# DIYer22/calibrating

Measured on AMD Instinct MI355X. Metric: stereo pairs/s at 1920x1080 numDisparities=128, higher is better.
Workload: dtype int16; 1 GPU; cv2.StereoSGBM-equivalent disparity of 1920x1080 rectified RGB pairs, numDisparities=128 blockSize=5 mode=MODE_SGBM(5 paths), median3 on, speckle off; batches_in_flight_per_gpu=2, parallelism=pairs sharded over 1 GPU(s), no data-path collective

## Files before the change

### calibrating_amd/csrc/common.hpp

```cpp
#pragma once

#include <hip/hip_runtime.h>

#include <cstdarg>
#include <cstdint>
#include <cstdio>

#include "../../include/calibrating_amd.h"
#include "../../include/calibrating_amd_experimental.h"

namespace camd {

void set_error(const char* fmt, ...);

#define CAMD_HIP(call)                                                                  \
    do {                                                                                \
        hipError_t e_ = (call);                                                         \
        if (e_ != hipSuccess) {                                                         \
            camd::set_error("%s failed: %s (%s:%d)", #call, hipGetErrorString(e_),      \
                            __FILE__, __LINE__);                                        \
            return CAMD_ERR_HIP;                                                        \
        }                                                                               \
    } while (0)

#define CAMD_LAUNCH_CHECK()                                                             \
    do {                                                                                \
        hipError_t e_ = hipGetLastError();                                              \
        if (e_ != hipSuccess) {                                                         \
            camd::set_error("kernel launch failed: %s (%s:%d)", hipGetErrorString(e_),  \
                            __FILE__, __LINE__);                                        \
            return CAMD_ERR_HIP;                                                        \
        }                                                                               \
    } while (0)

typedef unsigned short u16x2_t __attribute__((ext_vector_type(2)));
typedef short s16x2_t __attribute__((ext_vector_type(2)));

__device__ __forceinline__ uint32_t pk_min_u16(uint32_t a, uint32_t b)
{
    return __builtin_bit_cast(uint32_t, __builtin_elementwise_min(__builtin_bit_cast(u16x2_t, a),
                                                                  __builtin_bit_cast(u16x2_t, b)));
}
__device__ __forceinline__ uint32_t pk_max_u16(uint32_t a, uint32_t b)
{
    return __builtin_bit_cast(uint32_t, __builtin_elementwise_max(__builtin_bit_cast(u16x2_t, a),
                                                                  __builtin_bit_cast(u16x2_t, b)));
}
__device__ __forceinline__ uint32_t pk_add_u16(uint32_t a, uint32_t b)
{
    return __builtin_bit_cast(uint32_t, __builtin_bit_cast(u16x2_t, a) + __builtin_bit_cast(u16x2_t, b));
}
__device__ __forceinline__ uint32_t pk_sub_u16(uint32_t a, uint32_t b)
{
    return __builtin_bit_cast(uint32_t, __builtin_bit_cast(u16x2_t, a) - __builtin_bit_cast(u16x2_t, b));
}
__device__ __forceinline__ uint32_t pk_min_i16(uint32_t a, uint32_t b)
{
    return __builtin_bit_cast(uint32_t, __builtin_elementwise_min(__builtin_bit_cast(s16x2_t, a),
                                                                  __builtin_bit_cast(s16x2_t, b)));
}
__device__ __forceinline__ uint32_t pk_max_i16(uint32_t a, uint32_t b)
{
    return __builtin_bit_cast(uint32_t, __builtin_elementwise_max(__builtin_bit_cast(s16x2_t, a),
                                                                  __builtin_bit_cast(s16x2_t, b)));
}
__device__ __forceinline__ uint32_t pk_subsat_u16(uint32_t a, uint32_t b)
{
    return __builtin_bit_cast(uint32_t, __builtin_elementwise_sub_sat(__builtin_bit_cast(u16x2_t, a),
                                                                      __builtin_bit_cast(u16x2_t, b)));
}
__device__ __forceinline__ uint32_t pk_addsat_i16(uint32_t a, uint32_t b)
{
    return __builtin_bit_cast(uint32_t, __builtin_elementwise_add_sat(__builtin_bit_cast(s16x2_t, a),
                                                                      __builtin_bit_cast(s16x2_t, b)));
}
__device__ __forceinline__ uint32_t pk_subsat_i16(uint32_t a, uint32_t b)
{
    return __builtin_bit_cast(uint32_t, __builtin_elementwise_sub_sat(__builtin_bit_cast(s16x2_t, a),
                                                                      __builtin_bit_cast(s16x2_t, b)));
}
__device__ __forceinline__ uint32_t pk_mad_sat_u16(uint32_t a, uint32_t b, uint32_t c)
{
    uint32_t r;
    asm("v_pk_mad_u16 %0, %1, %2, %3 clamp" : "=v"(r) : "v"(a), "v"(b), "v"(c));
    return r;
}
__device__ __forceinline__ uint32_t pk_lshr_u16(uint32_t a, uint32_t sh_pk)
{
    return __builtin_bit_cast(uint32_t, __builtin_bit_cast(u16x2_t, a) >> __builtin_bit_cast(u16x2_t, sh_pk));
}
__device__ __forceinline__ uint32_t alignbit16(uint32_t hi, uint32_t lo)
{
    return __builtin_amdgcn_alignbit(hi, lo, 16);
}
__device__ __forceinline__ uint32_t dup16(uint32_t v) { return (v & 0xffffu) | (v << 16); }

enum : int {
    DPP_QUAD_XOR1 = 0xB1,
    DPP_QUAD_XOR2 = 0x4E,
    DPP_ROW_SHL1 = 0x101,
    DPP_ROW_SHR1 = 0x111,
    DPP_WAVE_SHL1 = 0x130,
    DPP_WAVE_SHR1 = 0x138,
    DPP_ROW_MIRROR = 0x140,
    DPP_ROW_HALF_MIRROR = 0x141
};

template <int CTRL>
__device__ __forceinline__ uint32_t dpp_mov(uint32_t old, uint32_t src)
{
    return (uint32_t)__builtin_amdgcn_update_dpp((int)old, (int)src, CTRL, 0xf, 0xf, false);
}

template <int LANES>
__device__ __forceinline__ uint32_t group_min_pk_u16(uint32_t v)
{
    if (LANES >= 2) v = pk_min_u16(v, dpp_mov<DPP_QUAD_XOR1>(v, v));
    if (LANES >= 4) v = pk_min_u16(v, dpp_mov<DPP_QUAD_XOR2>(v, v));
    if (LANES >= 8) v = pk_min_u16(v, dpp_mov<DPP_ROW_HALF_MIRROR>(v, v));
    if (LANES >= 16) v = pk_min_u16(v, dpp_mov<DPP_ROW_MIRROR>(v, v));
    return v;
}
template <int LANES>
__device__ __forceinline__ uint32_t group_min_u32(uint32_t v)
{
    if (LANES >= 2) v = min(v, dpp_mov<DPP_QUAD_XOR1>(v, v));
    if (LANES >= 4) v = min(v, dpp_mov<DPP_QUAD_XOR2>(v, v));
    if (LANES >= 8) v = min(v, dpp_mov<DPP_ROW_HALF_MIRROR>(v, v));
    if (LANES >= 16) v = min(v, dpp_mov<DPP_ROW_MIRROR>(v, v));
    return v;
}
template <int LANES>
__device__ __forceinline__ uint32_t group_max_u32(uint32_t v)
{
    if (LANES >= 2) v = max(v, dpp_mov<DPP_QUAD_XOR1>(v, v));
    if (LANES >= 4) v = max(v, dpp_mov<DPP_QUAD_XOR2>(v, v));
    if (LANES >= 8) v = max(v, dpp_mov<DPP_ROW_HALF_MIRROR>(v, v));
    if (LANES >= 16) v = max(v, dpp_mov<DPP_ROW_MIRROR>(v, v));
    return v;
}
template <int LANES>
__device__ __forceinline__ uint32_t group_or_u32(uint32_t v)
{
    if (LANES >= 2) v |= dpp_mov<DPP_QUAD_XOR1>(v, v);
    if (LANES >= 4) v |= dpp_mov<DPP_QUAD_XOR2>(v, v);
    if (LANES >= 8) v |= dpp_mov<DPP_ROW_HALF_MIRROR>(v, v);
    if (LANES >= 16) v |= dpp_mov<DPP_ROW_MIRROR>(v, v);
    return v;
}

template <int CTRL>
__device__ __forceinline__ uint32_t dpp_perm(uint32_t src)
{
    return (uint32_t)__builtin_amdgcn_update_dpp(0, (int)src, CTRL, 0xf, 0xf, true);
}
template <int LANES>
__device__ __forceinline__ uint32_t group_min_u32_full(uint32_t v)
{
    if (LANES >= 2) v = min(v, dpp_perm<DPP_QUAD_XOR1>(v));
    if (LANES >= 4) v = min(v, dpp_perm<DPP_QUAD_XOR2>(v));
    if (LANES >= 8) v = min(v, dpp_perm<DPP_ROW_HALF_MIRROR>(v));
    if (LANES >= 16) v = min(v, dpp_perm<DPP_ROW_MIRROR>(v));
    return v;
}
template <int LANES>
__device__ __forceinline__ uint32_t group_min_dup16(uint32_t pk)
{
    uint32_t v = pk_min_u16(pk, alignbit16(pk, pk));
    return group_min_u32_full<LANES>(v);
}

constexpr int CAMD_MAX_P2 = 24000;
constexpr int CAMD_MAX_FTZERO = 127;
static_assert(CAMD_MAX_P2 < 0x8000, "P1 < P2 must fit a signed 16-bit half: sgm_step adds them with plain 32-bit adds");
static_assert(2 * CAMD_MAX_FTZERO + 63 < 0x8000, "a pixel cost must fit a 16-bit half");

static inline int div_up(long long a, long long b) { return (int)((a + b - 1) / b); }

enum { INTER_BITS = 5, INTER_TAB_SIZE = 1 << INTER_BITS };

static inline int images_per_group(long long groups_per_image, int batch)
{
    int zb = batch < 16 ? batch : 16;
    while (zb > 1 && groups_per_image * div_up(batch, zb) < 4096) zb = (zb + 1) / 2;
    return zb;
}

static inline bool float_type_ok(int value_type) { return value_type == CAMD_VALUE_F64 || value_type == CAMD_VALUE_F32; }

}
```

### calibrating_amd/csrc/sgbm.hip

```cpp
#include "common.hpp"

#include <cstdlib>
#include <cstring>
#include <new>

namespace camd {

static constexpr uint32_t SENT_PK = 0x7fff7fffu;
static constexpr int MAX_COST = 32767;
static constexpr int CAMD_MULTI_MAX_BATCH = 8;

struct Geom {
    int W, H, cn;
    int minD, D, Dp;
    int minX1, W1;
    int SW2;
    int P1, P2, uniq, d12;
    int ftzero;
    int lanes, nr;
    int mode, npaths;
    uint32_t uniq_magic;
    int speckleWindowSize, speckleRange;
};

}
#include "sgbm_split.hpp"
#include "sgbm_cost.hpp"
#include "sgbm_scan.hpp"
#include "sgbm_band.hpp"
#include "sgbm_exact.hpp"
namespace camd {

int launch_median3(const int16_t* src, size_t src_pitch_e, size_t src_stride_e, int16_t* dst,
                   size_t dst_pitch_e, size_t dst_stride_e, int w, int h, int batch, hipStream_t st);
int launch_speckle(int16_t* img, size_t pitch_e, size_t stride_e, int w, int h, int new_val, int max_size,
                   int max_diff, void* ws, size_t ws_bytes, int batch, hipStream_t st, bool* clean);
size_t speckle_ws_bytes(int w, int h, int batch);

enum Stage { ST_COST = 0, ST_HSUM, ST_VSUM, ST_SCAN, ST_SCAN2, ST_WTA, ST_POST, ST_SPECKLE, ST_COUNT };
static const char* kStageNames[ST_COUNT] = {"cost", "hsum", "vsum", "scan", "scan_last", "wta", "median", "speckle"};

}

struct camd_sgbm {
    camd::Geom g;
    camd::Geom ga;
    camd::CostRanges cr;
    int stripe_sz;
    int16_t* rawv;
    uint32_t* cost_ovf;
    uint32_t* cost_neg;
    bool may_overflow;
    int exact_cap;
    int32_t* Lx;
    int way3_simd_lanes;
    camd_sgbm_params params;
    int max_batch;
    size_t vol_elems;
    size_t raw_stride, rawv_stride;
    size_t speckle_bytes;
    uint16_t *C, *S;
    int16_t* raw;
    void* speckle_ws;
    bool speckle_clean;
    hipStream_t speckle_stream;
    bool band_ok;
    int path;
    int keep_S;
    int cost_path;
    int saturate;
    int phases;
    int nbands, nchunks;
    size_t erec_stride;
    unsigned long long* E;
    uint32_t *flags, *ticket, *err, *keys;
    uint32_t* xbar;
    int num_cus;
    int persist_cost, persist_row;
    uint32_t* err_host;
    int16_t* d1;
    uint32_t epoch;
    uint16_t* Smulti;
    int smulti_cap;
    int last_batch;
    bool profiling;
    hipEvent_t ev[camd::ST_COUNT + 1];
    bool ev_ok;
};

namespace camd {

static int normalise(const camd_sgbm_params* p, int width, int height, int cn, Geom* g)
{
    if (!p) { set_error("params is NULL"); return CAMD_ERR_BAD_ARG; }
    if (width <= 0 || height <= 0 || (cn != 1 && cn != 3)) {
        set_error("need width, height > 0 and 1 or 3 channels (got %d x %d x %d)", width, height, cn);
        return CAMD_ERR_BAD_ARG;
    }
    if (p->numDisparities <= 0) { set_error("numDisparities must be > 0"); return CAMD_ERR_BAD_ARG; }
    if (p->mode < CAMD_MODE_SGBM || p->mode > CAMD_MODE_HH4) {
        set_error("mode %d unknown (MODE_SGBM=0, MODE_HH=1, MODE_SGBM_3WAY=2, MODE_HH4=3)", p->mode);
        return CAMD_ERR_BAD_ARG;
    }
    memset(g, 0, sizeof(*g));
    g->W = width; g->H = height; g->cn = cn;
    g->minD = p->minDisparity; g->D = p->numDisparities;
    int maxD = g->minD + g->D;
    g->minX1 = maxD > 0 ? maxD : 0;
    int maxX1 = width + (g->minD < 0 ? g->minD : 0);
    g->W1 = maxX1 - g->minX1;
    g->uniq = p->uniquenessRatio >= 0 ? p->uniquenessRatio : 10;
    g->uniq_magic = (g->uniq <= 98) ? (uint32_t)((1ull << 32) / (unsigned)(100 - g->uniq) + 1) : 0u;
    g->d12 = p->disp12MaxDiff > 0 ? p->disp12MaxDiff : 1;
    g->P1 = p->P1 > 0 ? p->P1 : 2;
    int P2 = p->P2 > 0 ? p->P2 : 5;
    g->P2 = P2 > g->P1 + 1 ? P2 : g->P1 + 1;
    int bs = p->blockSize > 0 ? p->blockSize : 5;
    g->SW2 = bs / 2;
    if (p->mode == CAMD_MODE_SGBM_3WAY && p->blockSize <= 0) g->SW2 = 1;
    g->ftzero = (p->preFilterCap > 15 ? p->preFilterCap : 15) | 1;
    g->mode = p->mode;
    g->npaths = p->mode == CAMD_MODE_HH ? 8 : (p->mode == CAMD_MODE_HH4 ? 4 : (p->mode == CAMD_MODE_SGBM_3WAY ? 3 : 5));
    g->speckleWindowSize = p->speckleWindowSize;
    g->speckleRange = p->speckleRange;
    if (2 * g->SW2 + 1 > HSUM_RING) {
        set_error("blockSize %d > %d not implemented", bs, HSUM_RING - 1);
        return CAMD_ERR_UNSUPPORTED;
    }
    if (g->P2 > CAMD_MAX_P2 || g->ftzero > CAMD_MAX_FTZERO) {
        set_error("P2 = %d / preFilterCap = %d outside the int16 regime the kernels implement", g->P2,
                  p->preFilterCap);
        return CAMD_ERR_UNSUPPORTED;
    }
    if (g->W1 > 0 && g->W1 <= g->SW2) {
        set_error("only %d matchable columns for blockSize %d: cv2.StereoSGBM's result is undefined there "
                  "(needs width - numDisparities > blockSize / 2)", g->W1, bs);
        return CAMD_ERR_UNSUPPORTED;
    }
    if (g->D > 512) { set_error("numDisparities %d > 512 not implemented", g->D); return CAMD_ERR_UNSUPPORTED; }
    if (g->D > 64) {
        g->lanes = 16;
        g->nr = (g->D <= 256 && p->mode != CAMD_MODE_SGBM_3WAY) ? (g->D + 31) / 32 : 4 * ((g->D + 127) / 128);
    }
    else if (g->D > 32) { g->lanes = 8; g->nr = 4; }
    else if (g->D > 16) { g->lanes = 4; g->nr = 4; }
    else { g->lanes = 2; g->nr = 4; }
    g->Dp = g->lanes * 2 * g->nr;
    return CAMD_OK;
}

static size_t align_up(size_t v, size_t a) { return (v + a - 1) / a * a; }

static int cost_ranges(const Geom& g, int block_size_raw, CostRanges* cr, int* stripe_sz, int* max_rows)
{
    if (g.mode != CAMD_MODE_SGBM_3WAY) {
        cr->n = 1;
        cr->start[0] = 0; cr->rows[0] = g.H;
        for (int i = 1; i < 4; i++) { cr->start[i] = 0; cr->rows[i] = 0; }
        *stripe_sz = g.H;
        *max_rows = g.H;
        return CAMD_OK;
    }
    const int ns = 4, sz = div_up(g.H, ns), ov = (block_size_raw / 2 + 1) + div_up(sz, 10);
    cr->n = ns;
    *stripe_sz = sz;
    *max_rows = 0;
    for (int s = 0; s < ns; s++) {
        int a = s * sz - ov, b = (s + 1) * sz < g.H ? (s + 1) * sz : g.H;
        if (s > 0 && s * sz < g.H && a < 0) {
            set_error("image height %d too small for MODE_SGBM_3WAY with blockSize %d (a stripe of %d rows needs a warm-up "
                      "of %d rows above it)", g.H, block_size_raw, sz, ov);
            return CAMD_ERR_UNSUPPORTED;
        }
        a = a < 0 ? 0 : (a > g.H ? g.H : a);
        cr->start[s] = a;
        cr->rows[s] = b > a ? b - a : 0;
        if (cr->rows[s] > *max_rows) *max_rows = cr->rows[s];
    }
    return CAMD_OK;
}

static bool params_may_overflow(const Geom& g)
{
    const long long K = 2 * g.SW2 + 1;
    return K * K * g.cn * (2 * g.ftzero + 63) + g.P2 > 32767;
}

static double pair_work(const Geom& g) { return ((double)g.H * g.W1 * g.Dp) / (1080.0 * 1792.0 * 128.0); }
static double auto_concurrent_limit(const Geom& g) { return g.mode == CAMD_MODE_HH ? 8.0 : 4.0; }
static int band_fill_workgroups(const Geom& g) { return (g.mode == CAMD_MODE_HH || g.mode == CAMD_MODE_HH4) ? 300 : 150; }
static int auto_concurrent_pairs(const Geom& g, bool band_ok, int max_batch, int nbands)
{
    int cap = max_batch < CAMD_MULTI_MAX_BATCH ? max_batch : CAMD_MULTI_MAX_BATCH;
    int n;
    if (band_ok && nbands > 0) n = (band_fill_workgroups(g) - 1) / nbands;
    else n = (int)(auto_concurrent_limit(g) / pair_work(g));
    if (n < 1) n = 1;
    return n < cap ? n : cap;
}

static bool band_supported(const Geom& g)
{
    const bool shape = g.W1 > 0 && g.nr <= 8;
    return shape && (g.mode == CAMD_MODE_SGBM_3WAY || g.uniq <= 99);
}

#define CAMD_FOR_SHAPE(g, M)                      \
    do {                                          \
        if ((g).lanes == 2) M(2, 4);              \
        else if ((g).lanes == 4) M(4, 4);         \
        else if ((g).lanes == 8) M(8, 4);         \
        else switch ((g).nr) {                    \
            case 3: M(16, 3); break;              \
            case 4: M(16, 4); break;              \
            case 5: M(16, 5); break;              \
            case 6: M(16, 6); break;              \
            case 7: M(16, 7); break;              \
            case 8: M(16, 8); break;              \
            case 12: M(16, 12); break;            \
            default: M(16, 16);                   \
        }                                         \
    } while (0)
#define CAMD_FOR_BAND_SHAPE(g, M)                 \
    do {                                          \
        if ((g).lanes == 2) M(2, 4);              \
        else if ((g).lanes == 4) M(4, 4);         \
        else if ((g).lanes == 8) M(8, 4);         \
        else switch ((g).nr) {                    \
            case 3: M(16, 3); break;              \
            case 4: M(16, 4); break;              \
            case 5: M(16, 5); break;              \
            case 6: M(16, 6); break;              \
            case 7: M(16, 7); break;              \
            default: M(16, 8);                    \
        }                                         \
    } while (0)

static int invalid_disp(const Geom& g) { return (g.minD - 1) * 16; }

static const int kDirs8[8][2] = {{1, 0}, {1, 1}, {0, 1}, {-1, 1}, {-1, 0}, {1, -1}, {0, -1}, {-1, -1}};

static int fill_scan_dirs(const Geom& g, const int (*dirs)[2], int ndirs, size_t dir_stride, ScanDirs* sd)
{
    int maxlines = 0;
    for (int i = 0; i < 8; i++) {
        const int k = i < ndirs ? i : 0;
        sd->dx[i] = dirs[k][0];
        sd->dy[i] = dirs[k][1];
        sd->nlines[i] = sd->dy[i] == 0 ? g.H : (sd->dx[i] == 0 ? g.W1 : g.W1 + g.H - 1);
        if (i < ndirs && sd->nlines[i] > maxlines) maxlines = sd->nlines[i];
    }
    sd->dir_stride = dir_stride;
    return maxlines;
}

template <bool FIRST>
static int launch_scan(const camd_sgbm* h, const int (*dirs)[2], int ndirs, uint16_t* S, size_t dir_stride,
                       int batch, hipStream_t st)
{
    const Geom& g = h->ga;
    ScanDirs sd;
    const int maxlines = fill_scan_dirs(g, dirs, ndirs, dir_stride, &sd);
    dim3 grid(div_up((long long)maxlines * g.lanes, 256), batch, ndirs);
    const bool pad = g.Dp != g.D;
#define CAMD_SCAN(LN, NVV)                                                                                  \
    do {                                                                                                    \
        if (pad) hipLaunchKernelGGL((k_scan<LN, NVV, FIRST, true>), grid, dim3(256), 0, st, h->C, S, g, sd, \
                                    h->vol_elems);                                                          \
        else hipLaunchKernelGGL((k_scan<LN, NVV, FIRST, false>), grid, dim3(256), 0, st, h->C, S, g, sd,    \
                                h->vol_elems);                                                              \
    } while (0)
    CAMD_FOR_SHAPE(g, CAMD_SCAN);
#undef CAMD_SCAN
    CAMD_LAUNCH_CHECK();
    return CAMD_OK;
}

static int launch_wta(const camd_sgbm* h, const uint16_t* S, int nvol, size_t dir_stride, int16_t* disp,
                      size_t pitch_e, size_t stride_e, int batch, hipStream_t st)
{
    const Geom& g = h->ga;
    const int tie_lanes = g.mode == CAMD_MODE_SGBM_3WAY ? h->way3_simd_lanes : 0;
    dim3 grid(g.H, batch);
    size_t lds = (size_t)g.W * 6;
    lds = align_up(lds, 16);
#define CAMD_WTA(LN, NVV)                                                                       \
    hipLaunchKernelGGL((k_wta<LN, NVV>), grid, dim3(256), lds, st, S, disp, pitch_e, stride_e, g, \
                       h->vol_elems, nvol, dir_stride, tie_lanes)
    CAMD_FOR_SHAPE(g, CAMD_WTA);
#undef CAMD_WTA
    CAMD_LAUNCH_CHECK();
    return CAMD_OK;
}

static int launch_band(camd_sgbm* h, int sx, int sy, bool full, int mode, int batch, hipStream_t st, bool diag = true,
                       bool tie8 = false)
{
    const Geom& g = h->ga;
    BandArgs a;
    a.C = h->C; a.S = h->S; a.E = h->E; a.flags = h->flags; a.ticket = h->ticket; a.err = h->err;
    a.keys = h->keys; a.d1 = h->d1; a.vol_stride = h->vol_elems; a.erec_stride = h->erec_stride;
    a.sx = sx; a.sy = sy; a.nbands = h->nbands; a.nchunks = h->nchunks; a.npairs = batch;
    a.epoch = ++h->epoch;
    a.write_S = h->keep_S;
    CAMD_HIP(hipMemsetAsync(h->ticket, 0, 4, st));
    dim3 grid(full ? h->nbands * batch : div_up((long long)batch * g.H, BAND_THREADS / g.lanes)), block(BAND_BLOCK);
    const bool pad = g.Dp != g.D;
#define CAMD_BAND(LN, NRR, FF, MM, DG)                                                                          \
    do {                                                                                                        \
        if (pad || (NRR) % 4 != 0) hipLaunchKernelGGL((k_band<LN, NRR, FF, MM, true, DG>), grid, block, 0, st, a, g); \
        else hipLaunchKernelGGL((k_band<LN, ((NRR) % 4 ? 4 : (NRR)), FF, MM, false, DG>), grid, block, 0, st, a, g);   \
    } while (0)
#define CAMD_BAND_F0T(LN, NRR) CAMD_BAND(LN, NRR, true, 0, true)
#define CAMD_BAND_F2T(LN, NRR) CAMD_BAND(LN, NRR, true, 2, true)
#define CAMD_BAND_F0F(LN, NRR) CAMD_BAND(LN, NRR, true, 0, false)
#define CAMD_BAND_F2F(LN, NRR) CAMD_BAND(LN, NRR, true, 2, false)
#define CAMD_BAND_R2(LN, NRR) CAMD_BAND(LN, NRR, false, 2, true)
#define CAMD_BAND_R1(LN, NRR) CAMD_BAND(LN, NRR, false, 1, true)
    if (full && mode == 0 && diag) CAMD_FOR_BAND_SHAPE(g, CAMD_BAND_F0T);
    else if (full && mode == 2 && diag) CAMD_FOR_BAND_SHAPE(g, CAMD_BAND_F2T);
    else if (full && mode == 0) CAMD_FOR_BAND_SHAPE(g, CAMD_BAND_F0F);
    else if (full && mode == 2) CAMD_FOR_BAND_SHAPE(g, CAMD_BAND_F2F);
    else if (!full && mode == 2 && tie8) {
#define CAMD_BAND_TIE(LN, NRR)                                                                                  \
    do {                                                                                                        \
        if (pad) hipLaunchKernelGGL((k_band<LN, NRR, false, 2, true, true, true>), grid, block, 0, st, a, g);   \
        else hipLaunchKernelGGL((k_band<LN, NRR, false, 2, false, true, true>), grid, block, 0, st, a, g);      \
    } while (0)
        if (g.lanes == 16 && g.nr == 4) CAMD_BAND_TIE(16, 4);
        else if (g.lanes == 16) CAMD_BAND_TIE(16, 8);
        else if (g.lanes == 8) CAMD_BAND_TIE(8, 4);
        else if (g.lanes == 4) CAMD_BAND_TIE(4, 4);
        else CAMD_BAND_TIE(2, 4);
#undef CAMD_BAND_TIE
    }
    else if (!full && mode == 2 && h->persist_row > 0 && g.lanes == 16 && g.nr == 4) {
        const dim3 pgrid(h->persist_row * (h->num_cus > 0 ? h->num_cus : 256));
        if (pad) hipLaunchKernelGGL((k_band_row_persist<16, 4, true>), pgrid, block, 0, st, a, g);
        else hipLaunchKernelGGL((k_band_row_persist<16, 4, false>), pgrid, block, 0, st, a, g);
    }
    else if (!full && mode == 2) CAMD_FOR_BAND_SHAPE(g, CAMD_BAND_R2);
    else if (!full && mode == 1) CAMD_FOR_BAND_SHAPE(g, CAMD_BAND_R1);
    else { set_error("band pass (full %d, mode %d) not instantiated", (int)full, mode); return CAMD_ERR_UNSUPPORTED; }
#undef CAMD_BAND_F0T
#undef CAMD_BAND_F2T
#undef CAMD_BAND_F0F
#undef CAMD_BAND_F2F
#undef CAMD_BAND_R2
#undef CAMD_BAND_R1
#undef CAMD_BAND
    CAMD_LAUNCH_CHECK();
    return CAMD_OK;
}

__global__ __launch_bounds__(256) void k_poison_flagged(int16_t* __restrict__ raw, size_t stride_e, size_t n,
                                                        const uint32_t* __restrict__ neg, uint32_t* __restrict__ err,
                                                        int invalid)
{
    const int vp = blockIdx.y;
    if (!neg[vp]) return;
    for (size_t i = (size_t)blockIdx.x * 256 + threadIdx.x; i < n; i += (size_t)gridDim.x * 256)
        raw[(size_t)vp * stride_e + i] = (int16_t)invalid;
    if (blockIdx.x == 0 && threadIdx.x == 0) atomicOr(err, 2u);
}

static int launch_exact(const camd_sgbm* h, int nvolumes, int16_t* dst, size_t stride_e, size_t n_e, hipStream_t st)
{
    const Geom& g = h->ga;
    static const int d_hh4[4][2] = {{0, 1}, {0, -1}, {1, 0}, {-1, 0}};
    static const int d_3way[3][2] = {{-1, 0}, {1, 0}, {0, 1}};
    const int (*dirs)[2] = g.mode == CAMD_MODE_HH4 ? d_hh4 : (g.mode == CAMD_MODE_SGBM_3WAY ? d_3way : kDirs8);
    const int nd = g.npaths;
    ScanDirs sd;
    fill_scan_dirs(g, dirs, nd, h->vol_elems, &sd);
    const bool way3 = g.mode == CAMD_MODE_SGBM_3WAY;
    ExactArgs a;
    a.C = reinterpret_cast<const int16_t*>(h->C);
    a.Lx = h->Lx;
    a.dst = dst;
    a.vol_stride = h->vol_elems;
    a.dst_stride_e = stride_e;
    a.dst_pitch_e = (size_t)g.W;
    a.dst_n = n_e;
    a.neg = h->cost_neg;
    a.bar = h->xbar;
    a.err = h->err;
    a.nvol = nvolumes;
    a.nd = nd;
    a.tie_lanes = way3 ? h->way3_simd_lanes : 0;
    a.combine = g.mode == CAMD_MODE_HH4 ? 1 : (way3 ? 2 : 0);
    a.min_as_int = g.mode == CAMD_MODE_HH4 ? 1 : 0;
    a.invalid = invalid_disp(g);
    CAMD_HIP(hipMemsetAsync(h->xbar, 0, 4, st));
    const size_t lds = align_up((size_t)g.W * 6, 16);
    const dim3 grid(h->num_cus > 0 ? h->num_cus : 256);
    Geom gg = g;
    void* kargs[] = {(void*)&a, (void*)&gg, (void*)&sd};
#define CAMD_XALL(LN, NRR)                                                                                          \
    do {                                                                                                            \
        const void* fn = way3 ? (const void*)k_exact_all<LN, NRR, true> : (const void*)k_exact_all<LN, NRR, false>; \
        if (hipLaunchCooperativeKernel(fn, grid, dim3(256), kargs, lds, st) != hipSuccess) {                        \
            (void)hipGetLastError();                                                                                \
            if (way3) hipLaunchKernelGGL((k_exact_all<LN, NRR, true>), grid, dim3(256), lds, st, a, g, sd);         \
            else hipLaunchKernelGGL((k_exact_all<LN, NRR, false>), grid, dim3(256), lds, st, a, g, sd);             \
        }                                                                                                           \
    } while (0)
    CAMD_FOR_SHAPE(g, CAMD_XALL);
#undef CAMD_XALL
    CAMD_LAUNCH_CHECK();
    return CAMD_OK;
}

static size_t smulti_bytes(const Geom& g, size_t vol_elems, int pairs) { return (size_t)g.npaths * pairs * vol_elems * 2; }
static size_t lx_bytes(const Geom& g, size_t vol_elems) { return (size_t)g.npaths * vol_elems * 4; }

struct WorkspacePlan {
    CostRanges cr;
    int stripe_sz, vrows;
    size_t vol_elems;
    size_t raw_stride, rawv_stride;
    bool band_ok, may_overflow;
    int nbands, nchunks, smulti_cap;
    size_t erec_stride;
    size_t C, S;
    size_t rawv, raw;
    size_t vol_flags;
    size_t ticket;
    size_t speckle;
    size_t E, band_flags, keys, d1;
    size_t Smulti;
    size_t Lx;
    size_t ticket_unreported;
    size_t rawv_unallocated;
};

static int plan_workspace(const Geom& g, const camd_sgbm_params& p, int max_batch, WorkspacePlan* w)
{
    memset(w, 0, sizeof(*w));
    const int rc = cost_ranges(g, p.blockSize, &w->cr, &w->stripe_sz, &w->vrows);
    if (rc != CAMD_OK) return rc;
    const bool way3 = g.mode == CAMD_MODE_SGBM_3WAY, matchable = g.W1 > 0;
    const size_t w1 = matchable ? (size_t)g.W1 : 0, nvol = (size_t)max_batch * w->cr.n;
    w->vol_elems = align_up((size_t)w->vrows * w1 * g.Dp * 2, 256) / 2;
    w->raw_stride = align_up((size_t)g.H * g.W * 2, 256) / 2;
    w->rawv_stride = align_up((size_t)w->vrows * g.W * 2, 256) / 2;
    w->C = w->S = nvol * w->vol_elems * 2;
    const size_t rawv = way3 ? nvol * w->rawv_stride * 2 : 0;
    w->rawv = matchable ? rawv : 0;
    w->rawv_unallocated = matchable ? 0 : rawv;
    w->raw = (size_t)max_batch * w->raw_stride * 2;
    w->vol_flags = nvol * 8;
    w->ticket = 16;
    w->ticket_unreported = 8;
    w->speckle = g.speckleWindowSize > 0 ? speckle_ws_bytes(g.W, g.H, max_batch) : 0;
    w->band_ok = band_supported(g);
    if (w->band_ok) {
        w->nbands = div_up(w->vrows, BAND_THREADS / g.lanes);
        w->nchunks = div_up(g.W1, BAND_CHUNK);
        w->erec_stride = band_erec_stride(g.W1, g.lanes, (g.nr + 3) / 4);
        const size_t npix = nvol * w->vrows * g.W;
        w->E = nvol * w->nbands * w->erec_stride * 8;
        w->band_flags = nvol * w->nbands * w->nchunks * 4;
        w->keys = npix * 4;
        w->d1 = npix * 2;
    }
    w->may_overflow = params_may_overflow(g);
    if (matchable) {
        w->smulti_cap = way3 ? 0 : auto_concurrent_pairs(g, w->band_ok, max_batch, w->nbands);
        w->Smulti = smulti_bytes(g, w->vol_elems, w->smulti_cap);
        if (w->may_overflow) w->Lx = lx_bytes(g, w->vol_elems);
    }
    return CAMD_OK;
}

#define CAMD_TRY(call) do { const int rc_ = (call); if (rc_ != CAMD_OK) return rc_; } while (0)

static int mark(camd_sgbm* h, int i, hipStream_t st)
{
    if (h->profiling && h->ev_ok) CAMD_HIP(hipEventRecord(h->ev[i], st));
    return CAMD_OK;
}
static int mark_rest(camd_sgbm* h, int first, hipStream_t st)
{
    for (int i = first; i <= ST_COUNT; i++) CAMD_TRY(mark(h, i, st));
    return CAMD_OK;
}

enum CostForm { COST_CHUNKED, COST_SATURATING, COST_RESIDENT };
struct CostShape {
    int nw, ndblk, nstrips;
    int nchunks, rows_per_chunk;
    size_t lds;
};
static CostShape cost_launch_shape(const camd_sgbm* h, int vbatch, CostForm form)
{
    const Geom& g = h->g;
    const int K = 2 * g.SW2 + 1, rows = h->ga.H;
    CostShape s;
    const int maxw = g.cn == 3 ? CAMD_COST_MAX_WAVES_RGB : CAMD_COST_MAX_WAVES_GRAY;
    s.nw = g.Dp / COST_DL < 4 ? 4 : (g.Dp / COST_DL < maxw ? g.Dp / COST_DL : maxw);
    s.ndblk = div_up(g.Dp, s.nw * COST_DL);
    s.nstrips = div_up(g.W1, 64 - (K - 1));
    s.lds = cost_lds_bytes(g.cn, s.nw);
    int nchunks = 1;
    if (form != COST_SATURATING) {
        const long long per_chunk = (long long)s.nstrips * s.ndblk * vbatch;
        const int maxc = rows / 32 > 1 ? rows / 32 : 1;
        nchunks = form == COST_RESIDENT ? div_up(24LL * h->persist_cost * (h->num_cus > 0 ? h->num_cus : 256), per_chunk)
                                        : div_up(8192, per_chunk);
        nchunks = nchunks < 1 ? 1 : (nchunks > maxc ? maxc : nchunks);
        const long long places = 256LL * (s.nw <= 8 ? 3 : 1);
        if (form == COST_CHUNKED && per_chunk * nchunks < 6 * places) {
            long long best = -1;
            for (int nc = 1; nc <= maxc; nc++) {
                const long long cost = (long long)div_up(per_chunk * nc, places) * (div_up(rows, nc) + K - 1);
                if (best < 0 || cost < best) { best = cost; nchunks = nc; }
            }
        }
    }
    s.rows_per_chunk = div_up(rows, nchunks);
    s.nchunks = div_up(rows, s.rows_per_chunk);
    return s;
}

static int launch_cost(camd_sgbm* h, const uint8_t* left, const uint8_t* right, size_t pitch, size_t image_stride,
                       int vbatch, bool sat_kernel, uint32_t* ovf, int thresh, hipStream_t st)
{
    const Geom& g = h->g;
    const int K = 2 * g.SW2 + 1;
    CostShape s = cost_launch_shape(h, vbatch, sat_kernel ? COST_SATURATING : COST_CHUNKED);
    const bool resident = h->persist_cost > 0 && !sat_kernel && !ovf && h->cr.n == 1 && (K == 5 || K == 3) &&
                          g.D % (s.nw * COST_DL) == 0;
    if (resident) s = cost_launch_shape(h, vbatch, COST_RESIDENT);
    const dim3 grid(s.nstrips, s.nchunks * s.ndblk, vbatch), block(64 * s.nw);
    if (resident) {
        uint32_t* tk = h->ticket + 3;
        const int nx = s.nstrips, ny = s.nchunks * s.ndblk, nitems = nx * ny * vbatch;
        const dim3 pgrid(h->persist_cost * (h->num_cus > 0 ? h->num_cus : 256));
#define CAMD_COSTP(CNN, KK) hipLaunchKernelGGL((k_cost_persist<CNN, KK>), pgrid, block, s.lds, st, left, right, pitch, image_stride, \
                                               h->C, g, s.rows_per_chunk, s.nchunks, h->vol_elems, h->cr, tk, nx, ny, nitems)
        if (g.cn == 1) { if (K == 5) CAMD_COSTP(1, 5); else CAMD_COSTP(1, 3); }
        else { if (K == 5) CAMD_COSTP(3, 5); else CAMD_COSTP(3, 3); }
#undef CAMD_COSTP
        CAMD_LAUNCH_CHECK();
        return CAMD_OK;
    }
#define CAMD_COST(CNN, KK, SS)                                                                                          \
    hipLaunchKernelGGL((k_cost<CNN, KK, SS>), grid, block, s.lds, st, left, right, pitch, image_stride, h->C, g,        \
                       s.rows_per_chunk, s.nchunks, h->vol_elems, h->cr, ovf, thresh, h->cost_neg)
#define CAMD_COST_K(CNN)                                                                         \
    switch (K) {                                                                                 \
        case 1: CAMD_COST(CNN, 1, false); break;                                                 \
        case 3: CAMD_COST(CNN, 3, false); break;                                                 \
        case 5: if (sat_kernel) CAMD_COST(CNN, 5, true); else CAMD_COST(CNN, 5, false); break;   \
        case 7: if (sat_kernel) CAMD_COST(CNN, 7, true); else CAMD_COST(CNN, 7, false); break;   \
        case 9: if (sat_kernel) CAMD_COST(CNN, 9, true); else CAMD_COST(CNN, 9, false); break;   \
        default: if (sat_kernel) CAMD_COST(CNN, 11, true); else CAMD_COST(CNN, 11, false);       \
    }
    if (g.cn == 1) { CAMD_COST_K(1) } else { CAMD_COST_K(3) }
#undef CAMD_COST_K
#undef CAMD_COST
    CAMD_LAUNCH_CHECK();
    return CAMD_OK;
}

static int launch_hsum(camd_sgbm* h, const uint8_t* left, const uint8_t* right, size_t pitch, size_t image_stride,
                       int batch, hipStream_t st)
{
    const Geom& g = h->g;
    int nseg = div_up(g.W1, HSUM_SEG), ndblk = div_up(g.Dp, 64);
    dim3 grid(nseg, g.H, batch), block(64 * ndblk);
    const int es = g.cn == 1 ? 4 : 12;
    const size_t maxr = HSUM_SEG + 2 * g.SW2 + ndblk * 64 + 2, maxl = HSUM_SEG + 2 * g.SW2 + 2;
    size_t lds = ((maxr + maxl) * es + (size_t)ndblk * (2 * g.SW2 + 1) * 64) * 4;
#define CAMD_HSUM(CNN, KK)                                                                                        \
    hipLaunchKernelGGL((k_hsum<CNN, KK>), grid, block, lds, st, left, right, pitch, image_stride, h->S, g, ndblk, \
                       h->vol_elems)
#define CAMD_HSUM_K(CNN)                                \
    switch (2 * g.SW2 + 1) {                            \
        case 1: CAMD_HSUM(CNN, 1); break;               \
        case 3: CAMD_HSUM(CNN, 3); break;               \
        case 5: CAMD_HSUM(CNN, 5); break;               \
        case 7: CAMD_HSUM(CNN, 7); break;               \
        case 9: CAMD_HSUM(CNN, 9); break;               \
        case 11: CAMD_HSUM(CNN, 11); break;             \
        default: CAMD_HSUM(CNN, 0);                     \
    }
    if (g.cn == 1) { CAMD_HSUM_K(1) } else { CAMD_HSUM(3, 0); }
#undef CAMD_HSUM_K
#undef CAMD_HSUM
    CAMD_LAUNCH_CHECK();
    return CAMD_OK;
}
static int launch_vsum(camd_sgbm* h, bool sat, int batch, hipStream_t st)
{
    const Geom& g = h->g;
    const int K = 2 * g.SW2 + 1;
    size_t rowv = (size_t)g.W1 * (g.Dp / 8);
    const uint4* hs4 = reinterpret_cast<const uint4*>(h->S);
    uint4* c4 = reinterpret_cast<uint4*>(h->C);
    const size_t ring_lds = (size_t)K * 256 * sizeof(uint4);
    if (sat) {
        const dim3 vgrid(div_up((long long)rowv, 256), 1, batch);
        hipLaunchKernelGGL(k_vsum<true>, vgrid, dim3(256), ring_lds, st, hs4, c4, g, h->vol_elems / 8, g.H);
    } else {
        const dim3 vgrid(div_up((long long)rowv, 256), div_up(g.H, VSUM_ROWS), batch);
        switch (K) {
#define CAMD_VSUM(KK) case KK: hipLaunchKernelGGL((k_vsum_reg<KK>), vgrid, dim3(256), 0, st, hs4, c4, g, h->vol_elems / 8); break
            CAMD_VSUM(1); CAMD_VSUM(3); CAMD_VSUM(5); CAMD_VSUM(7); CAMD_VSUM(9); CAMD_VSUM(11);
#undef CAMD_VSUM
            default:
                hipLaunchKernelGGL(k_vsum<false>, vgrid, dim3(256), ring_lds, st, hs4, c4, g, h->vol_elems / 8, VSUM_ROWS);
        }
    }
    CAMD_LAUNCH_CHECK();
    return CAMD_OK;
}

static int run_cost(camd_sgbm* h, const uint8_t* left, const uint8_t* right, size_t pitch, size_t image_stride, int batch,
                    hipStream_t st)
{
    const Geom& g = h->g;
    const int K = 2 * g.SW2 + 1;
    const bool may_overflow = h->may_overflow;
    const bool sat = h->saturate && may_overflow;
    const bool way3 = g.mode == CAMD_MODE_SGBM_3WAY;
    const int vbatch = batch * h->cr.n;
    const bool fused = K <= 11 && (h->cost_path != CAMD_COST_SPLIT || way3);
    const bool do_cost = (h->phases & 1) != 0;
    if (fused && do_cost) {
        const int tbound = K * g.cn * (2 * g.ftzero + 63);
        const bool two_stage = sat && (long long)K * tbound + g.P2 <= 65535;
        if (may_overflow) CAMD_HIP(hipMemsetAsync(h->cost_neg, 0, (size_t)vbatch * 4, st));
        if (h->persist_cost > 0) CAMD_HIP(hipMemsetAsync(h->ticket + 3, 0, 4, st));
        if (two_stage) {
            CAMD_HIP(hipMemsetAsync(h->cost_ovf, 0, (size_t)vbatch * 4, st));
            CAMD_TRY(launch_cost(h, left, right, pitch, image_stride, vbatch, false, h->cost_ovf, 32767 - tbound, st));
            CAMD_TRY(launch_cost(h, left, right, pitch, image_stride, vbatch, true, h->cost_ovf, -1, st));
        } else {
            CAMD_TRY(launch_cost(h, left, right, pitch, image_stride, vbatch, sat, nullptr, -1, st));
        }
    }
    CAMD_TRY(mark(h, ST_HSUM, st));
    if (!fused && do_cost) CAMD_TRY(launch_hsum(h, left, right, pitch, image_stride, batch, st));
    CAMD_TRY(mark(h, ST_VSUM, st));
    if (!fused && do_cost) CAMD_TRY(launch_vsum(h, sat, batch, st));
    if (do_cost && may_overflow && !(fused && sat)) {
        if (!fused) CAMD_HIP(hipMemsetAsync(h->cost_neg, 0, (size_t)vbatch * 4, st));
        hipLaunchKernelGGL(k_flag_below, dim3(512, 1, vbatch), dim3(256), 0, st, reinterpret_cast<const int16_t*>(h->C),
                           h->ga, h->vol_elems, h->cr, h->cost_neg);
        CAMD_LAUNCH_CHECK();
    }
    return CAMD_OK;
}

static int choose_path(const camd_sgbm* h, int batch)
{
    const Geom& g = h->g;
    const bool way3 = g.mode == CAMD_MODE_SGBM_3WAY;
    const long long band_wgs = (long long)h->nbands * batch * h->cr.n;
    int path = h->path;
    if (path == CAMD_PATH_AUTO) {
        if (h->band_ok && band_wgs >= band_fill_workgroups(g)) path = CAMD_PATH_BAND;
        else path = CAMD_PATH_CONCURRENT;
    }
    if (way3) {
        if (h->path == CAMD_PATH_AUTO) path = batch * pair_work(g) < 2.5 ? CAMD_PATH_SCAN : CAMD_PATH_BAND;
        else if (path != CAMD_PATH_SCAN) path = CAMD_PATH_BAND;
    }
    if (path == CAMD_PATH_BAND && !h->band_ok) path = CAMD_PATH_SCAN;
    if (path == CAMD_PATH_CONCURRENT && batch > h->smulti_cap)
        path = (h->band_ok && (h->path != CAMD_PATH_AUTO || band_wgs >= 128)) ? CAMD_PATH_BAND : CAMD_PATH_SCAN;
    if (h->path == CAMD_PATH_AUTO && path == CAMD_PATH_BAND && g.lanes <= 4 && band_wgs < 128) path = CAMD_PATH_SCAN;
    return path;
}

static bool way3_inline(const camd_sgbm* h) { return h->way3_simd_lanes == 1 || h->g.D % 8 == 0; }
static bool stops_before_last_pass(const camd_sgbm* h, int path)
{
    return path == CAMD_PATH_BAND && h->g.mode != CAMD_MODE_SGBM_3WAY && !(h->phases & 4);
}
static int launch_wta_init(camd_sgbm* h, const Geom& ga, int nimages, hipStream_t st)
{
    const size_t npix = (size_t)nimages * ga.H * ga.W;
    hipLaunchKernelGGL(k_wta_init, dim3(div_up((long long)npix, 256)), dim3(256), 0, st, h->keys, h->d1, npix, invalid_disp(ga));
    CAMD_LAUNCH_CHECK();
    return CAMD_OK;
}

static int run_aggregation(camd_sgbm* h, int batch, int path, hipStream_t st)
{
    const Geom& g = h->g;
    const bool way3 = g.mode == CAMD_MODE_SGBM_3WAY;
    const int vbatch = batch * h->cr.n;
    if (path == CAMD_PATH_BAND && way3) {
        if (way3_inline(h)) CAMD_TRY(launch_wta_init(h, h->ga, vbatch, st));
        CAMD_TRY(launch_band(h, +1, +1, true, 0, vbatch, st, false));
        CAMD_TRY(mark(h, ST_SCAN2, st));
        if (way3_inline(h)) CAMD_TRY(launch_band(h, -1, +1, false, 2, vbatch, st, true, h->way3_simd_lanes == 8));
        else CAMD_TRY(launch_band(h, -1, +1, false, 1, vbatch, st));
    } else if (path == CAMD_PATH_BAND) {
        if (h->phases & 2) {
            CAMD_TRY(launch_wta_init(h, g, batch, st));
            CAMD_TRY(launch_band(h, +1, +1, true, 0, batch, st, g.mode != CAMD_MODE_HH4));
        }
        CAMD_TRY(mark(h, ST_SCAN2, st));
        if (stops_before_last_pass(h, path)) return CAMD_OK;
        if (g.mode == CAMD_MODE_HH4) CAMD_TRY(launch_band(h, -1, -1, true, 2, batch, st, false));
        else if (g.mode == CAMD_MODE_HH) CAMD_TRY(launch_band(h, -1, -1, true, 2, batch, st));
        else CAMD_TRY(launch_band(h, -1, +1, false, 2, batch, st));
    } else {
        static const int dirs4[4][2] = {{1, 0}, {0, 1}, {-1, 0}, {0, -1}};
        const int (*dirs)[2] = (g.mode == CAMD_MODE_HH4 || way3) ? dirs4 : kDirs8;
        if (path == CAMD_PATH_CONCURRENT) {
            CAMD_TRY(launch_scan<true>(h, dirs, g.npaths, h->Smulti, (size_t)h->smulti_cap * h->vol_elems, batch, st));
        } else {
            for (int i = 0; i < g.npaths; i++)
                CAMD_TRY(i == 0 ? launch_scan<true>(h, dirs + i, 1, h->S, 0, vbatch, st)
                                : launch_scan<false>(h, dirs + i, 1, h->S, 0, vbatch, st));
        }
        CAMD_TRY(mark(h, ST_SCAN2, st));
    }
    return CAMD_OK;
}

static int redo_flagged(camd_sgbm* h, int16_t* dst, size_t stride_e, size_t n_e, int nvolumes, hipStream_t st)
{
    if (!h->may_overflow) return CAMD_OK;
    if (h->exact_cap) return launch_exact(h, nvolumes, dst, stride_e, n_e, st);
    hipLaunchKernelGGL(k_poison_flagged, dim3(64, nvolumes), dim3(256), 0, st, dst, stride_e, n_e, h->cost_neg, h->err,
                       invalid_disp(h->g));
    CAMD_LAUNCH_CHECK();
    CAMD_HIP(hipMemcpyAsync(h->err_host, h->err, 4, hipMemcpyDeviceToHost, st));
    return CAMD_OK;
}

static int launch_lrcheck(camd_sgbm* h, const Geom& ga, int16_t* out, size_t stride_e, int nimages, hipStream_t st)
{
    hipLaunchKernelGGL(k_lrcheck, dim3(div_up(div_up(ga.W, 2), 256), div_up(ga.H, LRCHECK_ROWS), nimages), dim3(256), 0, st, h->d1,
                       h->keys, out, (size_t)ga.W, stride_e, ga, h->err);
    CAMD_LAUNCH_CHECK();
    return CAMD_OK;
}

static int run_winners(camd_sgbm* h, int batch, int path, hipStream_t st)
{
    const Geom& g = h->g;
    const bool band = path == CAMD_PATH_BAND;
    if (g.mode == CAMD_MODE_SGBM_3WAY) {
        const int vbatch = batch * h->cr.n;
        if (band && way3_inline(h)) CAMD_TRY(launch_lrcheck(h, h->ga, h->rawv, h->rawv_stride, vbatch, st));
        else CAMD_TRY(launch_wta(h, h->S, 1, 0, h->rawv, (size_t)g.W, h->rawv_stride, vbatch, st));
        CAMD_TRY(redo_flagged(h, h->rawv, h->rawv_stride, (size_t)h->ga.H * g.W, vbatch, st));
        hipLaunchKernelGGL(k_gather_stripes, dim3(div_up(g.W, 256), g.H, batch), dim3(256), 0, st, h->rawv, h->rawv_stride,
                           h->raw, h->raw_stride, g.W, g.H, h->stripe_sz, h->cr, band ? h->err : nullptr,
                           (h->may_overflow && !h->exact_cap) ? h->cost_neg : nullptr, invalid_disp(g));
        CAMD_LAUNCH_CHECK();
        if (band) CAMD_HIP(hipMemcpyAsync(h->err_host, h->err, 4, hipMemcpyDeviceToHost, st));
        return CAMD_OK;
    }
    if (band) {
        CAMD_TRY(launch_lrcheck(h, g, h->raw, h->raw_stride, batch, st));
        CAMD_HIP(hipMemcpyAsync(h->err_host, h->err, 4, hipMemcpyDeviceToHost, st));
    } else if (path == CAMD_PATH_CONCURRENT) {
        CAMD_TRY(launch_wta(h, h->Smulti, g.npaths, (size_t)h->smulti_cap * h->vol_elems, h->raw, (size_t)g.W, h->raw_stride, batch, st));
    } else {
        CAMD_TRY(launch_wta(h, h->S, 1, 0, h->raw, (size_t)g.W, h->raw_stride, batch, st));
    }
    return redo_flagged(h, h->raw, h->raw_stride, (size_t)g.H * g.W, batch, st);
}

static int run_post(camd_sgbm* h, int16_t* disp, size_t dpe, size_t dse, int batch, hipStream_t st)
{
    const Geom& g = h->g;
    CAMD_TRY(launch_median3(h->raw, g.W, h->raw_stride, disp, dpe, dse, g.W, g.H, batch, st));
    CAMD_TRY(mark(h, ST_SPECKLE, st));
    if (g.speckleWindowSize > 0) {
        if (h->speckle_stream != st) { h->speckle_clean = false; h->speckle_stream = st; }
        CAMD_TRY(launch_speckle(disp, dpe, dse, g.W, g.H, invalid_disp(g), g.speckleWindowSize, 16 * g.speckleRange,
                                h->speckle_ws, h->speckle_bytes, batch, st, &h->speckle_clean));
    }
    return mark(h, ST_COUNT, st);
}

}

using namespace camd;

extern "C" {

size_t camd_sgbm_workspace_bytes(const camd_sgbm_params* p, int width, int height, int channels,
                                 int max_batch)
{
    Geom g;
    WorkspacePlan w;
    if (normalise(p, width, height, channels, &g) != CAMD_OK || max_batch <= 0) return 0;
    if (plan_workspace(g, *p, max_batch, &w) != CAMD_OK) return 0;
    return w.C + w.S + w.rawv + w.raw + w.vol_flags + w.ticket + w.speckle + w.E + w.band_flags + w.keys + w.d1 + w.Smulti +
           w.Lx - w.ticket_unreported + w.rawv_unallocated;
}

int camd_sgbm_create(const camd_sgbm_params* p, int width, int height, int channels, int max_batch,
                     camd_sgbm** out)
{
    if (!out) { set_error("out is NULL"); return CAMD_ERR_BAD_ARG; }
    *out = nullptr;
    Geom g;
    int rc = normalise(p, width, height, channels, &g);
    if (rc != CAMD_OK) return rc;
    if (max_batch <= 0) { set_error("max_batch must be > 0"); return CAMD_ERR_BAD_ARG; }
    rc = camd_device_ok();
    if (rc != CAMD_OK) return rc;
    WorkspacePlan w;
    rc = plan_workspace(g, *p, max_batch, &w);
    if (rc != CAMD_OK) return rc;
    if (g.mode == CAMD_MODE_SGBM_3WAY && 2 * g.SW2 + 1 > 11) {
        set_error("MODE_SGBM_3WAY is implemented for blockSize <= 11");
        return CAMD_ERR_UNSUPPORTED;
    }
    camd_sgbm* h = new (std::nothrow) camd_sgbm();
    if (!h) { set_error("out of host memory"); return CAMD_ERR_NOMEM; }
    memset(h, 0, sizeof(*h));
    h->g = g;
    h->params = *p;
    h->max_batch = max_batch;
    h->way3_simd_lanes = 8;
    h->cr = w.cr;
    h->stripe_sz = w.stripe_sz;
    h->ga = g;
    h->ga.H = w.vrows;
    h->vol_elems = w.vol_elems;
    h->raw_stride = w.raw_stride;
    h->rawv_stride = w.rawv_stride;
    h->speckle_bytes = w.speckle;
    h->may_overflow = w.may_overflow;
    h->band_ok = w.band_ok;
    h->nbands = w.nbands;
    h->nchunks = w.nchunks;
    h->erec_stride = w.erec_stride;
    h->path = 0;
    h->saturate = 1;
    h->phases = 7;
    h->epoch = 0;
    h->persist_cost = h->persist_row = 0;
    hipError_t e = hipSuccess;
    auto alloc = [&e](auto** ptr, size_t bytes) {
        if (e == hipSuccess && bytes) e = hipMalloc((void**)ptr, bytes);
    };
    alloc(&h->C, w.C);
    if (e == hipSuccess && w.C && g.Dp != g.D) {
        hipStream_t fs = nullptr;
        e = hipStreamCreateWithFlags(&fs, hipStreamNonBlocking);
        if (e == hipSuccess) e = hipMemsetD16Async(h->C, (unsigned short)g.P2, w.C / 2, fs);
        if (e == hipSuccess) e = hipStreamSynchronize(fs);
        if (fs) (void)hipStreamDestroy(fs);
    }
    alloc(&h->S, w.S);
    alloc(&h->rawv, w.rawv);
    alloc(&h->raw, w.raw);
    alloc(&h->cost_ovf, w.vol_flags);
    h->cost_neg = h->cost_ovf ? h->cost_ovf + w.vol_flags / 8 : nullptr;
    if (e == hipSuccess) e = hipMemset(h->cost_ovf, 0, w.vol_flags);
    alloc(&h->ticket, w.ticket);
    if (e == hipSuccess) e = hipMemset(h->ticket, 0, w.ticket);
    h->err = h->ticket ? h->ticket + 1 : nullptr;
    h->xbar = h->ticket ? h->ticket + 2 : nullptr;
    {
        int dev = 0, ncu = 0;
        if (hipGetDevice(&dev) == hipSuccess && hipDeviceGetAttribute(&ncu, hipDeviceAttributeMultiprocessorCount, dev) == hipSuccess)
            h->num_cus = ncu;
        else
            (void)hipGetLastError();
    }
    if (e == hipSuccess) e = hipHostMalloc((void**)&h->err_host, 4, hipHostMallocDefault);
    if (e == hipSuccess) *h->err_host = 0;
    alloc(&h->speckle_ws, w.speckle);
    alloc(&h->E, w.E);
    alloc(&h->flags, w.band_flags);
    alloc(&h->keys, w.keys);
    alloc(&h->d1, w.d1);
    if (e == hipSuccess && w.band_flags) e = hipMemset(h->flags, 0, w.band_flags);
    if (e == hipSuccess) {
        int cap = w.smulti_cap;
        while (cap > 0) {
            if (hipMalloc((void**)&h->Smulti, smulti_bytes(g, h->vol_elems, cap)) == hipSuccess) break;
            (void)hipGetLastError();
            h->Smulti = nullptr;
            cap /= 2;
        }
        h->smulti_cap = cap;
        if (w.Lx) {
            if (hipMalloc((void**)&h->Lx, w.Lx) == hipSuccess) h->exact_cap = 1;
            else { (void)hipGetLastError(); h->Lx = nullptr; }
        }
    }
    if (e != hipSuccess) {
        set_error("workspace allocation failed: %s", hipGetErrorString(e));
        camd_sgbm_destroy(h);
        return e == hipErrorOutOfMemory ? CAMD_ERR_NOMEM : CAMD_ERR_HIP;
    }
    *out = h;
    return CAMD_OK;
}

static const char* device_error_text(uint32_t e)
{
    static const char* kRefused =
        "a cost volume left the int16 regime of the aggregation kernels (values below P2 after an overflow of the box "
        "sums) and the handle has no workspace for the exact path; the disparities of that pair were written as invalid";
    static const char* kTimeout =
        "a band-wavefront pass timed out waiting for its upstream band; the disparities of that call were written as "
        "invalid";
    static const char* kBoth =
        "a band-wavefront pass timed out waiting for its upstream band (the disparities of that call were written as "
        "invalid) AND a cost volume left the int16 regime of the aggregation kernels with no workspace for the exact "
        "path (that pair was written as invalid)";
    static const char* kBarrier =
        "the exact int path's grid barrier timed out (its workgroups were not all resident at once -- e.g. on a stream "
        "restricted to few compute units while other kernels held them); the disparities of the flagged pairs were written "
        "as invalid";
    if (e & 4u) return kBarrier;
    return (e & 3u) == 3u ? kBoth : ((e & 2u) ? kRefused : kTimeout);
}

int camd_sgbm_destroy(camd_sgbm* h)
{
    if (!h) return CAMD_OK;
    if (h->ev_ok)
        for (int i = 0; i <= ST_COUNT; i++) (void)hipEventDestroy(h->ev[i]);
    (void)hipFree(h->C); (void)hipFree(h->S);
    (void)hipFree(h->raw); (void)hipFree(h->rawv); (void)hipFree(h->speckle_ws); (void)hipFree(h->cost_ovf);
    (void)hipFree(h->E); (void)hipFree(h->flags); (void)hipFree(h->ticket); (void)hipFree(h->keys);
    (void)hipFree(h->d1); (void)hipFree(h->Smulti); (void)hipFree(h->Lx);
    if (h->err_host) (void)hipHostFree(h->err_host);
    delete h;
    return CAMD_OK;
}

int camd_sgbm_query(const camd_sgbm* h, int* width1, int* D, int* Dp, int* minX1)
{
    if (!h) { set_error("handle is NULL"); return CAMD_ERR_BAD_ARG; }
    if (width1) *width1 = h->g.W1;
    if (D) *D = h->g.D;
    if (Dp) *Dp = h->g.Dp;
    if (minX1) *minX1 = h->g.minX1;
    return CAMD_OK;
}

int camd_sgbm_set_option(camd_sgbm* h, int option, int value)
{
    if (!h) { set_error("handle is NULL"); return CAMD_ERR_BAD_ARG; }
    if (option == CAMD_OPT_PATH && value >= CAMD_PATH_AUTO && value <= CAMD_PATH_CONCURRENT) {
        if (value == CAMD_PATH_CONCURRENT && h->g.W1 > 0) {
            const int want = h->max_batch < CAMD_MULTI_MAX_BATCH ? h->max_batch : CAMD_MULTI_MAX_BATCH;
            if (want > h->smulti_cap) {
                CAMD_HIP(hipDeviceSynchronize());
                (void)hipFree(h->Smulti);
                h->Smulti = nullptr;
                h->smulti_cap = 0;
                hipError_t e = hipMalloc((void**)&h->Smulti, smulti_bytes(h->g, h->vol_elems, want));
                if (e != hipSuccess) {
                    (void)hipGetLastError();
                    set_error("no memory for %d x %d per-direction volumes", h->g.npaths, want);
                    return CAMD_ERR_NOMEM;
                }
                h->smulti_cap = want;
            }
        }
        h->path = value;
    }
    else if (option == CAMD_OPT_KEEP_S) h->keep_S = value != 0;
    else if (option == CAMD_OPT_COST && value >= CAMD_COST_AUTO && value <= CAMD_COST_SPLIT) h->cost_path = value;
    else if (option == CAMD_OPT_SATURATE) h->saturate = value != 0;
    else if (option == CAMD_OPT_3WAY_SIMD_LANES && (value == 1 || value == 8)) h->way3_simd_lanes = value;
    else if (option == CAMD_OPT_PHASES && value >= 1 && value <= 7) h->phases = value;
    else if (option == CAMD_OPT_RESIDENT && value >= 0 && (value >> 4) <= 4 && (value & 15) <= 4) {
        h->persist_cost = value >> 4;
        h->persist_row = value & 15;
    }
    else if (option == CAMD_OPT_EXACT) {
        if (value != 0 && !h->Lx && h->may_overflow) {
            if (hipMalloc((void**)&h->Lx, lx_bytes(h->g, h->vol_elems)) != hipSuccess) {
                (void)hipGetLastError();
                h->Lx = nullptr;
                set_error("no memory for the exact path's %d per-direction int volumes; the handle keeps refusing flagged pairs",
                          h->g.npaths);
                return CAMD_ERR_NOMEM;
            }
        }
        h->exact_cap = (value != 0 && h->Lx) ? 1 : 0;
    }
    else { set_error("unknown option %d / value %d", option, value); return CAMD_ERR_BAD_ARG; }
    return CAMD_OK;
}

int camd_sgbm_status(camd_sgbm* h, void* stream)
{
    if (!h) { set_error("handle is NULL"); return CAMD_ERR_BAD_ARG; }
    if (!h->err) return CAMD_OK;
    uint32_t e = 0;
    CAMD_HIP(hipMemcpyAsync(&e, h->err, 4, hipMemcpyDeviceToHost, (hipStream_t)stream));
    CAMD_HIP(hipStreamSynchronize((hipStream_t)stream));
    if (e) {
        CAMD_HIP(hipMemsetAsync(h->err, 0, 4, (hipStream_t)stream));
        if (h->err_host) *(volatile uint32_t*)h->err_host = 0;
        set_error("%s", device_error_text(e));
        return CAMD_ERR_HIP;
    }
    return CAMD_OK;
}

int camd_sgbm_set_profiling(camd_sgbm* h, int enable)
{
    if (!h) { set_error("handle is NULL"); return CAMD_ERR_BAD_ARG; }
    if (enable && !h->ev_ok) {
        for (int i = 0; i <= ST_COUNT; i++) CAMD_HIP(hipEventCreate(&h->ev[i]));
        h->ev_ok = true;
    }
    h->profiling = enable != 0;
    return CAMD_OK;
}
int camd_sgbm_num_stages(void) { return ST_COUNT; }
const char* camd_sgbm_stage_name(int i) { return i >= 0 && i < ST_COUNT ? kStageNames[i] : ""; }
int camd_sgbm_get_profile(camd_sgbm* h, float* ms, int n)
{
    if (!h || !ms) { set_error("NULL argument"); return CAMD_ERR_BAD_ARG; }
    if (!h->ev_ok || !h->profiling) { set_error("profiling not enabled"); return CAMD_ERR_BAD_ARG; }
    CAMD_HIP(hipEventSynchronize(h->ev[ST_COUNT]));
    for (int i = 0; i < n && i < ST_COUNT; i++) CAMD_HIP(hipEventElapsedTime(&ms[i], h->ev[i], h->ev[i + 1]));
    return CAMD_OK;
}

int camd_sgbm_compute(camd_sgbm* h, const uint8_t* left, const uint8_t* right, size_t pitch,
                      size_t image_stride, int16_t* disp, size_t disp_pitch, size_t disp_stride,
                      int batch, void* stream)
{
    if (!h || !left || !right || !disp) { set_error("NULL argument"); return CAMD_ERR_BAD_ARG; }
    const Geom& g = h->g;
    if (batch <= 0 || batch > h->max_batch) {
        set_error("batch %d outside [1, max_batch=%d]", batch, h->max_batch);
        return CAMD_ERR_BAD_ARG;
    }
    if (pitch < (size_t)g.W * g.cn || disp_pitch < (size_t)g.W * 2 || (disp_pitch & 1) || (disp_stride & 1)) {
        set_error("pitch too small or odd disparity pitch");
        return CAMD_ERR_BAD_ARG;
    }
    hipStream_t st = (hipStream_t)stream;
    if (h->err_host && *(volatile uint32_t*)h->err_host) {
        const uint32_t e = *(volatile uint32_t*)h->err_host;
        *(volatile uint32_t*)h->err_host = 0;
        CAMD_HIP(hipMemsetAsync(h->err, 0, 4, st));
        set_error("in an earlier compute on this handle: %s", device_error_text(e));
        return CAMD_ERR_HIP;
    }
    const size_t dpe = disp_pitch / 2, dse = disp_stride / 2;
    h->last_batch = batch;
    if (g.W1 <= 0) {
        hipLaunchKernelGGL(k_fill_s16, dim3(div_up(g.W, 256), g.H, batch), dim3(256), 0, st, disp, dpe, dse,
                           g.W, g.H, invalid_disp(g));
        CAMD_LAUNCH_CHECK();
        return CAMD_OK;
    }

    CAMD_TRY(mark(h, ST_COST, st));
    CAMD_TRY(run_cost(h, left, right, pitch, image_stride, batch, st));
    if (!(h->phases & 6)) return mark_rest(h, ST_SCAN, st);
    const int path = choose_path(h, batch);
    CAMD_TRY(mark(h, ST_SCAN, st));
    CAMD_TRY(run_aggregation(h, batch, path, st));
    if (stops_before_last_pass(h, path)) return mark_rest(h, ST_WTA, st);
    CAMD_TRY(mark(h, ST_WTA, st));
    CAMD_TRY(run_winners(h, batch, path, st));
    CAMD_TRY(mark(h, ST_POST, st));
    return run_post(h, disp, dpe, dse, batch, st);
}

int camd_sgbm_debug_copy(camd_sgbm* h, int which, int index, void* dst, void* stream)
{
    if (!h || !dst) { set_error("NULL argument"); return CAMD_ERR_BAD_ARG; }
    if (index < 0 || index >= h->max_batch) { set_error("index out of range"); return CAMD_ERR_BAD_ARG; }
    const Geom& g = h->g;
    hipStream_t st = (hipStream_t)stream;
    if (which == 0 || which == 1) {
        if (g.mode == CAMD_MODE_SGBM_3WAY) {
            set_error("MODE_SGBM_3WAY keeps its volumes per stripe: only which = 2 (raw disparity) is available");
            return CAMD_ERR_UNSUPPORTED;
        }
        if (g.W1 <= 0) return CAMD_OK;
        const uint16_t* src = (which == 0 ? h->C : h->S) + (size_t)index * h->vol_elems;
        CAMD_HIP(hipMemcpyAsync(dst, src, (size_t)g.H * g.W1 * g.Dp * 2, hipMemcpyDeviceToDevice, st));
    } else if (which == 2) {
        CAMD_HIP(hipMemcpyAsync(dst, h->raw + (size_t)index * h->raw_stride, (size_t)g.H * g.W * 2,
                                hipMemcpyDeviceToDevice, st));
    } else {
        set_error("which must be 0 (C), 1 (S) or 2 (raw disparity)");
        return CAMD_ERR_BAD_ARG;
    }
    return CAMD_OK;
}

}
```

### calibrating_amd/csrc/sgbm_band.hpp

```cpp
#pragma once

namespace camd {

#ifndef CAMD_BAND_NT
#define CAMD_BAND_NT 1
#endif
#ifndef CAMD_ROW_PERSIST_PRIO
#define CAMD_ROW_PERSIST_PRIO 3
#endif
#ifndef CAMD_BAND_MIN_WAVES
#define CAMD_BAND_MIN_WAVES 4
#endif
#ifndef CAMD_BAND_ROW_MIN_WAVES
#define CAMD_BAND_ROW_MIN_WAVES CAMD_BAND_MIN_WAVES
#endif
static constexpr int BAND_THREADS = 64 * 7;
static constexpr int BAND_BLOCK = BAND_THREADS + 64;
static constexpr int BAND_HELPER_WAVE = 7;
static constexpr int BAND_RING = 4;
#ifndef BAND_RING_ROWS
#define BAND_RING_ROWS 4
#endif
static constexpr int BAND_CHUNK = 16;
static constexpr uint32_t BAND_SPIN_LIMIT = 1u << 20;

struct BandArgs {
    const uint16_t* C;
    uint16_t* S;
    unsigned long long* E;
    uint32_t* flags;
    uint32_t* ticket;
    uint32_t* err;
    uint32_t* keys;
    int16_t* d1;
    size_t vol_stride;
    size_t erec_stride;
    int sx, sy, nbands, nchunks, npairs;
    uint32_t epoch;
    int write_S;
};

template <int LANES, int NR, bool PAD>
__device__ __forceinline__ uint32_t sgm_step(const uint32_t (&Lp)[NR], uint32_t delta, const uint32_t (&c)[NR],
                                             uint32_t (&L)[NR], const uint32_t (&keep)[NR],
                                             const uint32_t (&sent)[NR], uint32_t P1pk, uint32_t P2pk, int li,
                                             uint32_t& edge_lo, uint32_t& edge_hi)
{
    edge_lo = dpp_mov<DPP_ROW_SHR1>(edge_lo, Lp[NR - 1]);
    edge_hi = dpp_mov<DPP_ROW_SHL1>(edge_hi, Lp[0]);
    uint32_t prev_last = edge_lo, next_first = edge_hi;
    if (LANES < 16) {
        if (li == 0) prev_last = SENT_PK;
        if (li == LANES - 1) next_first = SENT_PK;
    }
    uint32_t m[NR + 1];
    m[0] = alignbit16(Lp[0], prev_last);
#pragma unroll
    for (int k = 1; k < NR; k++) m[k] = alignbit16(Lp[k], Lp[k - 1]);
    m[NR] = alignbit16(next_first, Lp[NR - 1]);
    uint32_t mn = SENT_PK;
#pragma unroll
    for (int k = 0; k < NR; k++) {
        uint32_t t = pk_min_u16(m[k], m[k + 1]) + P1pk;
        uint32_t l = c[k] - pk_subsat_u16(delta, pk_min_u16(Lp[k], t));
        if (PAD) l = (l & keep[k]) | sent[k];
        L[k] = l;
        mn = pk_min_u16(mn, l);
    }
    return group_min_dup16<LANES>(mn) + P2pk;
}


static inline size_t band_erec_stride(int W1, int lanes, int nq) { return (size_t)W1 * ((size_t)lanes * 6 * nq + 2); }

static constexpr uint32_t WTA_NONE = 0xffffffffu;
#ifndef CAMD_WTA_PADQ
#define CAMD_WTA_PADQ 4
#endif
template <int LANES> struct WtaPad { static constexpr int Q = (LANES * 16) % 128 == 0 ? CAMD_WTA_PADQ : 0; };

template <int LANES, int NR, bool TIE8 = false, int NTH = BAND_THREADS>
__device__ __forceinline__ void band_wta_step(const uint32_t (&s)[NR], const uint32_t (&dpk)[NR], uint4* wS,
                                              const Geom& g, int ctid, int grp, int li, int t, bool act,
                                              uint32_t& cap_key, uint32_t& cap_nb)
{
    constexpr int NQ = (NR + 3) / 4;
    static_assert(!TIE8 || NR % 4 == 0, "the 8-slot tie rule needs whole groups of 8 disparities per lane");
    uint32_t key = 0xffffffffu;
#pragma unroll
    for (int k = 0; k < NR; k++) {
        key = min(key, __builtin_amdgcn_perm(s[k], dpk[k], 0x05040100u));
        key = min(key, __builtin_amdgcn_perm(s[k], dpk[k], 0x07060302u));
    }
    key = group_min_u32_full<LANES>(key);
    const int minS = (int)(key >> 16);
    int best = (int)(key & 0xffffu);
    if (TIE8) {
        uint32_t kl = 0xffffffffu;
#pragma unroll
        for (int k = 0; k < NR; k++) {
            const uint32_t nd = ~dpk[k];
            kl = min(kl, __builtin_amdgcn_perm(s[k], nd, 0x05040100u));
            kl = min(kl, __builtin_amdgcn_perm(s[k], nd, 0x07060302u));
        }
        kl = group_min_u32_full<LANES>(kl);
        if (__any((int)(0xffffu - (kl & 0xffffu)) != best)) {
            uint32_t pos = 0xffffffffu;
#pragma unroll
            for (int e = 0; e < 8; e++) {
                uint32_t last = 0;
#pragma unroll
                for (int v = 0; v < NR / 4; v++) {
                    const uint32_t val = (e & 1) ? (s[4 * v + e / 2] >> 16) : (s[4 * v + e / 2] & 0xffffu);
                    const uint32_t d = (e & 1) ? (dpk[4 * v + e / 2] >> 16) : (dpk[4 * v + e / 2] & 0xffffu);
                    if ((int)d < g.D && (int)val == minS) last = d + 1;
                }
                last = group_max_u32<LANES>(last);
                if (last) pos = min(pos, last - 1);
            }
            best = (int)pos;
            key = ((uint32_t)minS << 16) | pos;
        }
    }
    constexpr int GST = LANES + WtaPad<LANES>::Q, WS_PLANE = (NTH / LANES) * GST;
    lds_st_regs<NR>(wS, grp * GST + li, WS_PLANE, s);
    const uint32_t bm1 = dup16((uint32_t)(best - 1));
    uint32_t far = 0xffffffffu;
#pragma unroll
    for (int k = 0; k < NR; k++) {
        const uint32_t w = pk_subsat_u16(0x00030003u, pk_sub_u16(dpk[k], bm1));
        far = pk_min_u16(far, pk_mad_sat_u16(w, 0xffffffffu, s[k]));
    }
    const int minfar = (int)(group_min_dup16<LANES>(far) & 0xffffu);
    const uint32_t uq = g.uniq <= 98 ? (uint32_t)(100 - g.uniq) : 1u;
    const bool ok = act && minS < MAX_COST && __umul24((uint32_t)minfar, uq) >= __umul24((uint32_t)minS, 100u);
    const uint16_t* gs = reinterpret_cast<const uint16_t*>(wS + grp * GST);
    auto slot_of = [](int d) {
        if (NQ == 1 && NR == 4) return d;
        const int ln = d / (2 * NR), w = d - ln * (2 * NR);
        return (w >> 3) * (WS_PLANE * 8) + ln * 8 + (w & 7);
    };
    const uint32_t Sm = gs[slot_of(max(best - 1, 0))], Sp = gs[slot_of(min(best + 1, LANES * 2 * NR - 1))];
    if (li == (t & (LANES - 1))) {
        cap_key = ok ? key : WTA_NONE;
        cap_nb = Sm | (Sp << 16);
    }
}

template <int LANES>
__device__ __forceinline__ void band_wta_flush(const BandArgs& a, const Geom& g, int pair, int y, int x,
                                               uint32_t& cap_key, uint32_t cap_nb)
{
    if (cap_key != WTA_NONE) {
        const int minS = (int)(cap_key >> 16);
        int d = (int)(cap_key & 0xffffu);
        const int x2 = x + g.minX1 - d - g.minD;
        const size_t ro = ((size_t)pair * g.H + y) * (size_t)g.W;
        atomicMin(a.keys + ro + x2, ((uint32_t)minS << 16) | (uint32_t)(0xffff - d));
        if (0 < d && d < g.D - 1) {
            const int Sm = (int)(cap_nb & 0xffffu), Sp = (int)(cap_nb >> 16);
            const int denom2 = max(Sm + Sp - 2 * minS, 1);
            const int num = (Sm - Sp) * 16 + denom2, den = denom2 * 2;
            int q = (int)((float)num * __frcp_rn((float)den));
            int r = num - q * den;
            if (num >= 0) {
                if (r < 0) q--;
                else if (r >= den) q++;
            } else {
                if (r > 0) q++;
                else if (r <= -den) q--;
            }
            d = d * 16 + q;
        } else
            d *= 16;
        a.d1[ro + x + g.minX1] = (int16_t)(d + g.minD * 16);
    }
    cap_key = WTA_NONE;
}

template <int LANES, int NR, bool FULL, int MODE, bool PAD, bool DIAG, bool TIE8, bool ALLW>
__device__ __forceinline__ void band_body(const BandArgs& a, const Geom& g, const int ticket)
{
    static_assert(!(FULL && ALLW), "the wavefront pass keeps its helper wave");
    constexpr int NQ = (NR + 3) / 4;
    constexpr int NTH = (!FULL && ALLW) ? BAND_BLOCK : BAND_THREADS;
    constexpr int R = NTH / LANES;
    constexpr int EVEC = 6 * NQ;
    constexpr int CPB = 64 / LANES;
    constexpr int RING = FULL ? BAND_RING : BAND_RING_ROWS;
    constexpr int SK = FULL ? 2 : 0;
    constexpr int XN = FULL ? BAND_THREADS * NQ : 1, EN = FULL ? 64 * NQ : 1;

    __shared__ uint4 xV[2][XN];
    __shared__ uint4 xD[2][XN];
    __shared__ uint4 xA[2][XN];
    __shared__ uint4 xdl[2][FULL ? R : 1];
    __shared__ uint4 eV[3][EN];
    __shared__ uint4 eD[3][EN];
    __shared__ uint4 eA[3][EN];
    __shared__ uint4 edl[3][FULL ? CPB : 1];
    __shared__ uint4 wS[MODE == 2 ? NQ * R * (LANES + WtaPad<LANES>::Q) : 1];

    const int band = FULL ? ticket / a.npairs : 0;
    const int wv = threadIdx.x >> 6;
    const bool helper = (FULL || !ALLW) && wv == BAND_HELPER_WAVE;
    if (!FULL && helper) return;
    const int ctid = (!FULL && ALLW) ? (int)threadIdx.x
                     : helper ? (int)(threadIdx.x & 63) : (((wv > BAND_HELPER_WAVE ? wv - 1 : wv) << 6) | (int)(threadIdx.x & 63));
    const int grp = ctid / LANES, li = ctid % LANES;
    const int W1 = g.W1, H = g.H;
    const long long grow = FULL ? 0 : min((long long)ticket * R + grp, (long long)a.npairs * H - 1);
    const int pair = FULL ? ticket % a.npairs : (int)(grow / H);
    const int row = FULL ? band * R + grp : (int)(grow % H);
    const bool rvalid = !helper && (FULL ? row < H : (long long)ticket * R + grp < (long long)a.npairs * H);
    const int y = a.sy > 0 ? row : H - 1 - row;
    const int glast = min(R, H - band * R) - 1;
    const bool has_prev = FULL && band > 0, has_next = FULL && band + 1 < a.nbands;
    const bool producer = !helper && has_next && grp == glast;
    const bool hduty = FULL && has_prev && helper;

    const uint32_t P1pk = dup16((uint32_t)g.P1), P2pk = dup16((uint32_t)g.P2);
    uint32_t keep[NR], sent[NR], dpk[NR];
#pragma unroll
    for (int k = 0; k < NR; k++) {
        int d0 = li * 2 * NR + 2 * k;
        dpk[k] = (uint32_t)d0 | ((uint32_t)(d0 + 1) << 16);
        uint32_t kp = (d0 < g.D ? 0xffffu : 0u) | (d0 + 1 < g.D ? 0xffff0000u : 0u);
        keep[k] = kp;
        sent[k] = ~kp & SENT_PK;
    }

    const size_t rowoff = (size_t)pair * a.vol_stride + ((size_t)(rvalid ? y : 0) * W1) * g.Dp + (size_t)li * (2 * NR);
    const uint16_t* Crow = a.C + rowoff;
    uint16_t* Srow = a.S + rowoff;
    auto cell_off = [&](int xi) -> size_t { return (size_t)(a.sx > 0 ? xi : W1 - 1 - xi) * g.Dp; };
    auto load_vec = [&](const uint16_t* p, uint32_t (&dst)[NR]) {
        if (CAMD_BAND_NT & 1) ld_regs_nt<NR>(p, dst);
        else ld_regs<NR>(p, dst);
    };
    auto lds_vec = [&](const uint4* p, int idx, int stride, uint32_t (&dst)[NR]) { lds_ld_regs<NR>(p, idx, stride, dst); };

    unsigned long long* Eout = a.E + ((size_t)pair * a.nbands + band) * a.erec_stride;
    const unsigned long long* Ein = a.E + ((size_t)pair * a.nbands + (band > 0 ? band - 1 : 0)) * a.erec_stride;
    const size_t edelta = (size_t)W1 * LANES * EVEC;
    uint32_t* Fout = a.flags + ((size_t)pair * a.nbands + band) * a.nchunks;
    const uint32_t* Fin = a.flags + ((size_t)pair * a.nbands + (band > 0 ? band - 1 : 0)) * a.nchunks;

    const int hl = threadIdx.x & 63;
    unsigned long long pend[EVEC], pdl[2];
#pragma unroll
    for (int k = 0; k < EVEC; k++) pend[k] = 0;
    pdl[0] = pdl[1] = 0;
    int edge_valid_upto = 0;
    bool dead = false;
    auto wait_cols = [&](int upto) {
        while (edge_valid_upto < upto) {
            const int chunk = edge_valid_upto / BAND_CHUNK;
            uint32_t spins = 0;
            while (!dead && __hip_atomic_load(Fin + chunk, __ATOMIC_RELAXED, __HIP_MEMORY_SCOPE_AGENT) != a.epoch) {
                __builtin_amdgcn_s_sleep(4);
                if (++spins > BAND_SPIN_LIMIT) {
                    atomicOr(a.err, 1u);
                    dead = true;
                }
            }
            edge_valid_upto = min((chunk + 1) * BAND_CHUNK, W1);
        }
    };
    auto fetch_batch = [&](int b) {
        const int col = b * CPB + hl / LANES;
        if (col < W1) {
            const unsigned long long* p = Ein + (size_t)col * (LANES * EVEC) + (hl % LANES);
#pragma unroll
            for (int k = 0; k < EVEC; k++)
                pend[k] = __hip_atomic_load(p + k * LANES, __ATOMIC_RELAXED, __HIP_MEMORY_SCOPE_AGENT);
            const unsigned long long* q = Ein + edelta + (size_t)col * 2;
            pdl[0] = __hip_atomic_load(q, __ATOMIC_RELAXED, __HIP_MEMORY_SCOPE_AGENT);
            pdl[1] = __hip_atomic_load(q + 1, __ATOMIC_RELAXED, __HIP_MEMORY_SCOPE_AGENT);
        }
    };
    auto park_batch = [&](int b) {
        const int slot = b % 3;
#pragma unroll
        for (int v = 0; v < NQ; v++) {
            eV[slot][v * 64 + hl] = make_uint4((uint32_t)pend[2 * v], (uint32_t)(pend[2 * v] >> 32),
                                               (uint32_t)pend[2 * v + 1], (uint32_t)(pend[2 * v + 1] >> 32));
            eD[slot][v * 64 + hl] =
                make_uint4((uint32_t)pend[2 * NQ + 2 * v], (uint32_t)(pend[2 * NQ + 2 * v] >> 32),
                           (uint32_t)pend[2 * NQ + 2 * v + 1], (uint32_t)(pend[2 * NQ + 2 * v + 1] >> 32));
            eA[slot][v * 64 + hl] =
                make_uint4((uint32_t)pend[4 * NQ + 2 * v], (uint32_t)(pend[4 * NQ + 2 * v] >> 32),
                           (uint32_t)pend[4 * NQ + 2 * v + 1], (uint32_t)(pend[4 * NQ + 2 * v + 1] >> 32));
        }
        if (hl % LANES == 0)
            edl[slot][hl / LANES] = make_uint4((uint32_t)pdl[0], (uint32_t)(pdl[0] >> 32), (uint32_t)pdl[1], 0u);
    };
    if (hduty) {
        wait_cols(min(CPB, W1));
        fetch_batch(0);
        park_batch(0);
        if (CPB < W1) {
            wait_cols(min(2 * CPB, W1));
            fetch_batch(1);
        }
    }

    uint32_t LH[NR];
    uint32_t VS[2][NR], DS[4][NR], dVs[2], dDs[4];
#pragma unroll
    for (int k = 0; k < NR; k++) {
        LH[k] = 0;
        VS[0][k] = VS[1][k] = 0;
        DS[0][k] = DS[1][k] = DS[2][k] = DS[3][k] = 0;
    }
    uint32_t dH = P2pk;
    uint32_t edge_lo = SENT_PK, edge_hi = SENT_PK;
    dVs[0] = dVs[1] = P2pk;
    dDs[0] = dDs[1] = dDs[2] = dDs[3] = P2pk;

    uint32_t cr[RING][NR], sr[RING][NR];
#pragma unroll
    for (int u = 0; u < RING; u++)
#pragma unroll
        for (int k = 0; k < NR; k++) { cr[u][k] = 0; sr[u][k] = 0; }
#pragma unroll
    for (int u = 0; u < RING - 1; u++) {
        const int xp = min(max(u - SK * grp, 0), W1 - 1);
        if (!helper) {
            load_vec(Crow + cell_off(xp), cr[u]);
            if (MODE != 0) load_vec(Srow + cell_off(xp), sr[u]);
        }
    }
    if (FULL) {
        if (!helper) {
#pragma unroll
            for (int v = 0; v < NQ; v++) {
                xV[1][v * BAND_THREADS + ctid] = make_uint4(0u, 0u, 0u, 0u);
                xD[1][v * BAND_THREADS + ctid] = make_uint4(0u, 0u, 0u, 0u);
                xA[1][v * BAND_THREADS + ctid] = make_uint4(0u, 0u, 0u, 0u);
            }
            if (li == 0) xdl[1][grp] = make_uint4(P2pk, P2pk, P2pk, 0u);
        }
        __syncthreads();
        if (!helper && grp == 0 && has_prev) {
            lds_vec(eV[0], li, 64, VS[1]);
            lds_vec(eD[0], li, 64, DS[3]);
            const uint4 dl = edl[0][0];
            dVs[1] = dl.x;
            dDs[3] = dl.y;
        }
    }

    const int nsteps = (W1 + SK * glast + RING - 1) / RING * RING;
    uint32_t cap_key = WTA_NONE, cap_nb = 0;
    auto duty_step = [&](int t) {
        const int b = t / CPB + 1;
        if (b * CPB < W1) park_batch(b);
        const int bn = b + 1;
        if (bn * CPB < W1) {
            wait_cols(min((bn + 1) * CPB, W1));
            fetch_batch(bn);
        }
    };
    if (FULL && helper) {
        for (int t = 0; t < nsteps; t++) {
            if (has_prev && (t % CPB) == 0) duty_step(t);
            asm volatile("s_waitcnt lgkmcnt(0)" ::: "memory");
#ifndef CAMD_BAND_DBG_NOBARRIER
            __builtin_amdgcn_s_barrier();
#endif
        }
        return;
    }
    for (int t0 = 0; t0 < nsteps; t0 += RING) {
#pragma unroll
        for (int u = 0; u < RING; u++) {
            const int t = t0 + u;
            const int xi = t - SK * grp;
            const bool act = rvalid && xi >= 0 && xi < W1;
            {
                constexpr int UP = (RING - 1);
                const int xp = min(max(xi + UP, 0), W1 - 1);
                load_vec(Crow + cell_off(xp), cr[(u + UP) % RING]);
                if (MODE != 0) load_vec(Srow + cell_off(xp), sr[(u + UP) % RING]);
            }
            const uint32_t(&cc)[NR] = cr[u];
            uint32_t An[NR], dAn = P2pk;
#pragma unroll
            for (int k = 0; k < NR; k++) An[k] = 0;
            if (FULL) {
                const int rb = (u & 1) ^ 1;
                if (grp > 0) {
                    lds_vec(xV[rb], ctid - LANES, BAND_THREADS, VS[u & 1]);
                    lds_vec(xD[rb], ctid - LANES, BAND_THREADS, DS[u & 3]);
                    lds_vec(xA[rb], ctid - LANES, BAND_THREADS, An);
                    const uint4 dl = xdl[rb][grp - 1];
                    dVs[u & 1] = dl.x;
                    dDs[u & 3] = dl.y;
                    dAn = dl.z;
                } else if (has_prev && xi + 1 < W1) {
                    const int col = xi + 1;
                    const int slot = (col / CPB) % 3, e = (col % CPB) * LANES + li;
                    lds_vec(eV[slot], e, 64, VS[u & 1]);
                    lds_vec(eD[slot], e, 64, DS[u & 3]);
                    lds_vec(eA[slot], e, 64, An);
                    const uint4 dl = edl[slot][col % CPB];
                    dVs[u & 1] = dl.x;
                    dDs[u & 3] = dl.y;
                    dAn = dl.z;
                }
            }
            const uint32_t(&Vin)[NR] = VS[(u + 1) & 1];
            const uint32_t(&Din)[NR] = DS[(u + 2) & 3];
            const uint32_t dV = dVs[(u + 1) & 1], dD = dDs[(u + 2) & 3];

            uint32_t LVo[NR], LDo[NR], LAo[NR], dVo = P2pk, dDo = P2pk, dAo = P2pk;
#pragma unroll
            for (int k = 0; k < NR; k++) { LVo[k] = 0; LDo[k] = 0; LAo[k] = 0; }
            if (act) {
                uint32_t s[NR];
#pragma unroll
                for (int k = 0; k < NR; k++) s[k] = MODE != 0 ? sr[u][k] : 0u;
                {
                    uint32_t L[NR];
                    dH = sgm_step<LANES, NR, PAD>(LH, dH, cc, L, keep, sent, P1pk, P2pk, li, edge_lo, edge_hi);
#pragma unroll
                    for (int k = 0; k < NR; k++) { LH[k] = L[k]; s[k] = pk_addsat_i16(s[k], L[k]); }
                }
                if (FULL) {
                    dVo = sgm_step<LANES, NR, PAD>(Vin, dV, cc, LVo, keep, sent, P1pk, P2pk, li, edge_lo, edge_hi);
#pragma unroll
                    for (int k = 0; k < NR; k++) s[k] = pk_addsat_i16(s[k], LVo[k]);
                    if (DIAG) {
                        dDo = sgm_step<LANES, NR, PAD>(Din, dD, cc, LDo, keep, sent, P1pk, P2pk, li, edge_lo, edge_hi);
#pragma unroll
                        for (int k = 0; k < NR; k++) s[k] = pk_addsat_i16(s[k], LDo[k]);
                        dAo = sgm_step<LANES, NR, PAD>(An, dAn, cc, LAo, keep, sent, P1pk, P2pk, li, edge_lo, edge_hi);
#pragma unroll
                        for (int k = 0; k < NR; k++) s[k] = pk_addsat_i16(s[k], LAo[k]);
                    }
                }
#if defined(CAMD_BAND_DBG_NOSTORE) && !defined(CAMD_MEASUREMENT_BUILD)
#error "CAMD_BAND_DBG_NOSTORE produces wrong results: measurement builds only (define CAMD_MEASUREMENT_BUILD too)"
#endif
#ifdef CAMD_BAND_DBG_NOSTORE
                if (s[0] == 0x12345678u) st_regs<NR>(Srow + cell_off(xi), s);
#else
                if (MODE != 2 || a.write_S) {
                    if (CAMD_BAND_NT & 2) st_regs_nt<NR>(Srow + cell_off(xi), s);
                    else st_regs<NR>(Srow + cell_off(xi), s);
                }
#endif
                if (MODE == 2) band_wta_step<LANES, NR, TIE8, NTH>(s, dpk, wS, g, ctid, grp, li, t, true, cap_key, cap_nb);
            }
            if (MODE == 2 && ((t & (LANES - 1)) == LANES - 1 || t == nsteps - 1)) {
                const int xc = xi - ((t & (LANES - 1)) - li);
                band_wta_flush<LANES>(a, g, pair, y, a.sx > 0 ? xc : W1 - 1 - xc, cap_key, cap_nb);
            }
            if (FULL) {
                const int wb = u & 1;
                lds_st_regs<NR>(xV[wb], ctid, BAND_THREADS, LVo);
                lds_st_regs<NR>(xD[wb], ctid, BAND_THREADS, LDo);
                lds_st_regs<NR>(xA[wb], ctid, BAND_THREADS, LAo);
                if (li == 0) xdl[wb][grp] = make_uint4(dVo, dDo, dAo, 0u);
                if (producer && act) {
                    unsigned long long* p = Eout + (size_t)xi * (LANES * EVEC) + li;
#pragma unroll
                    for (int k = 0; k < 2 * NQ; k++) {
                        if (2 * k >= NR) break;
                        __hip_atomic_store(p + k * LANES, (unsigned long long)LVo[2 * k] | ((unsigned long long)reg_or0<NR>(LVo, 2 * k + 1) << 32),
                                           __ATOMIC_RELAXED, __HIP_MEMORY_SCOPE_AGENT);
                        __hip_atomic_store(p + (2 * NQ + k) * LANES,
                                           (unsigned long long)LDo[2 * k] | ((unsigned long long)reg_or0<NR>(LDo, 2 * k + 1) << 32),
                                           __ATOMIC_RELAXED, __HIP_MEMORY_SCOPE_AGENT);
                        __hip_atomic_store(p + (4 * NQ + k) * LANES,
                                           (unsigned long long)LAo[2 * k] | ((unsigned long long)reg_or0<NR>(LAo, 2 * k + 1) << 32),
                                           __ATOMIC_RELAXED, __HIP_MEMORY_SCOPE_AGENT);
                    }
                    if (li == 0) {
                        unsigned long long* q = Eout + edelta + (size_t)xi * 2;
                        __hip_atomic_store(q, (unsigned long long)dVo | ((unsigned long long)dDo << 32), __ATOMIC_RELAXED,
                                           __HIP_MEMORY_SCOPE_AGENT);
                        __hip_atomic_store(q + 1, (unsigned long long)dAo, __ATOMIC_RELAXED, __HIP_MEMORY_SCOPE_AGENT);
                    }
                    if ((xi % BAND_CHUNK) == BAND_CHUNK - 1 || xi == W1 - 1) {
                        asm volatile("s_waitcnt vmcnt(0)" ::: "memory");
                        if (li == 0)
                            __hip_atomic_store(Fout + xi / BAND_CHUNK, a.epoch, __ATOMIC_RELAXED, __HIP_MEMORY_SCOPE_AGENT);
                    }
                }
                asm volatile("s_waitcnt lgkmcnt(0)" ::: "memory");
#if defined(CAMD_BAND_DBG_NOBARRIER) && !defined(CAMD_MEASUREMENT_BUILD)
#error "CAMD_BAND_DBG_NOBARRIER produces wrong results: measurement builds only (define CAMD_MEASUREMENT_BUILD too)"
#endif
#ifndef CAMD_BAND_DBG_NOBARRIER
                __builtin_amdgcn_s_barrier();
#endif
            }
        }
    }
}

template <int LANES, int NR, bool FULL, int MODE, bool PAD, bool DIAG = true, bool TIE8 = false>
__global__ __launch_bounds__(BAND_BLOCK, NR <= 4 ? (FULL ? CAMD_BAND_MIN_WAVES : CAMD_BAND_ROW_MIN_WAVES) : 2) void k_band(BandArgs a, Geom g)
{
    __shared__ uint32_t s_ticket;
    if (threadIdx.x == 0) s_ticket = atomicAdd(a.ticket, 1u);
    __syncthreads();
    band_body<LANES, NR, FULL, MODE, PAD, DIAG, TIE8, false>(a, g, (int)s_ticket);
}

template <int LANES, int NR, bool PAD, bool TIE8 = false>
__global__ __launch_bounds__(BAND_BLOCK, NR <= 4 ? CAMD_BAND_ROW_MIN_WAVES : 2) void k_band_row_persist(BandArgs a, Geom g)
{
    __shared__ uint32_t s_ticket;
    const long long rows = (long long)a.npairs * g.H;
#if CAMD_ROW_PERSIST_PRIO
    __builtin_amdgcn_s_setprio(CAMD_ROW_PERSIST_PRIO);
#endif
    for (;;) {
        if (threadIdx.x == 0) s_ticket = atomicAdd(a.ticket, 1u);
        __syncthreads();
        const int ticket = (int)s_ticket;
        __syncthreads();
        if ((long long)ticket * (BAND_BLOCK / LANES) >= rows) break;
        band_body<LANES, NR, false, 2, PAD, true, TIE8, true>(a, g, ticket);
    }
}

constexpr int LRCHECK_ROWS = 8;
__global__ __launch_bounds__(256) void k_lrcheck(const int16_t* __restrict__ d1, const uint32_t* __restrict__ keys,
                                                 int16_t* __restrict__ out, size_t out_pitch_e, size_t out_stride_e,
                                                 Geom g, const uint32_t* __restrict__ err)
{
    const int x0 = 2 * (blockIdx.x * 256 + threadIdx.x);
    if (x0 >= g.W) return;
    const bool two = x0 + 1 < g.W;
    const int ya = blockIdx.y * LRCHECK_ROWS, yb = min(ya + LRCHECK_ROWS, g.H), pair = blockIdx.z;
    const int INVALID_SCALED = (g.minD - 1) * 16;
    const bool poisoned = (*err & 1u) != 0;
    uint32_t both[LRCHECK_ROWS];
#pragma unroll
    for (int k = 0; k < LRCHECK_ROWS; k++) {
        const size_t ro = ((size_t)pair * g.H + min(ya + k, g.H - 1)) * (size_t)g.W;
        if (two) __builtin_memcpy(&both[k], d1 + ro + x0, 4);
        else both[k] = (uint16_t)d1[ro + x0];
    }
#pragma unroll
    for (int k = 0; k < LRCHECK_ROWS; k++) {
        const int y = ya + k;
        if (y >= yb) break;
        const size_t ro = ((size_t)pair * g.H + y) * (size_t)g.W;
        auto check = [&](int x, int v1) -> int {
            if (x >= g.minX1 && x < g.minX1 + g.W1 && v1 != INVALID_SCALED) {
                int _d = v1 >> 4, d_ = (v1 + 15) >> 4;
                int _x = x - _d, x_ = x - d_;
                bool bad = false;
                if (0 <= _x && _x < g.W) {
                    uint32_t kk = keys[ro + _x];
                    int v = kk == KEY_INIT ? INVALID_SCALED : (int)(0xffffu - (kk & 0xffffu)) + g.minD;
                    bad = v >= g.minD && abs(v - _d) > g.d12;
                }
                if (bad) {
                    bad = false;
                    if (0 <= x_ && x_ < g.W) {
                        uint32_t kk = keys[ro + x_];
                        int v = kk == KEY_INIT ? INVALID_SCALED : (int)(0xffffu - (kk & 0xffffu)) + g.minD;
                        bad = v >= g.minD && abs(v - d_) > g.d12;
                    }
                }
                if (bad) v1 = INVALID_SCALED;
            }
            return poisoned ? INVALID_SCALED : v1;
        };
        const uint32_t lo = (uint32_t)check(x0, (int)(int16_t)(both[k] & 0xffffu)) & 0xffffu;
        int16_t* o = out + (size_t)pair * out_stride_e + (size_t)y * out_pitch_e + x0;
        if (two) {
            const uint32_t r = lo | ((uint32_t)check(x0 + 1, (int)(int16_t)(both[k] >> 16)) << 16);
            __builtin_memcpy(o, &r, 4);
        } else
            *o = (int16_t)lo;
    }
}

__global__ __launch_bounds__(256) void k_wta_init(uint32_t* keys, int16_t* d1, size_t n, int invalid)
{
    size_t i = (size_t)blockIdx.x * 256 + threadIdx.x;
    if (i < n) {
        keys[i] = KEY_INIT;
        d1[i] = (int16_t)invalid;
    }
}

}
```

### calibrating_amd/csrc/sgbm_cost.hpp

```cpp
#pragma once

namespace camd {

static constexpr int COST_DL = 8;
#ifndef CAMD_COST_MAX_WAVES_RGB
#define CAMD_COST_MAX_WAVES_RGB 8
#endif
#ifndef CAMD_COST_MAX_WAVES_GRAY
#define CAMD_COST_MAX_WAVES_GRAY 16
#endif
#ifndef CAMD_COST_MIN_WAVES
#define CAMD_COST_MIN_WAVES 6
#endif
#ifndef CAMD_COST_LDS_FLOOR_RGB
#define CAMD_COST_LDS_FLOOR_RGB (41 * 1024)
#endif
#ifndef CAMD_COST_TSTORE
#define CAMD_COST_TSTORE 1
#endif

template <int N>
__device__ __forceinline__ uint32_t wave_shr(uint32_t v)
{
#pragma unroll
    for (int i = 0; i < N; i++) v = dpp_perm<DPP_WAVE_SHR1>(v);
    return v;
}

template <int K>
__device__ __forceinline__ uint32_t lane_window_sum(uint32_t p)
{
    if (K == 1) return p;
    const uint32_t w2 = p + wave_shr<1>(p);
    if (K == 3) return p + wave_shr<1>(w2);
    if (K == 5) {
        const uint32_t w4 = w2 + wave_shr<2>(w2);
        return p + wave_shr<1>(w4);
    }
    if (K == 7) {
        const uint32_t w3 = p + wave_shr<1>(w2);
        const uint32_t w6 = w3 + wave_shr<3>(w3);
        return p + wave_shr<1>(w6);
    }
    if (K == 9) {
        const uint32_t w4 = w2 + wave_shr<2>(w2);
        const uint32_t w8 = w4 + wave_shr<4>(w4);
        return p + wave_shr<1>(w8);
    }
    const uint32_t w4 = w2 + wave_shr<2>(w2);
    const uint32_t w5 = p + wave_shr<1>(w4);
    const uint32_t w10 = w5 + wave_shr<5>(w5);
    return p + wave_shr<1>(w10);
}


struct CostRanges {
    int n;
    int start[4], rows[4];
};

constexpr bool cost_tstore(int cn) { return (CAMD_COST_TSTORE & (cn == 1 ? 1 : 2)) != 0; }
static inline bool cost_tstore_shape(int cn, int nwaves) { return cost_tstore(cn) && 64 % nwaves == 0; }
static inline size_t cost_lds_bytes(int cn, int nwaves)
{
    const int es = cn == 1 ? 4 : 12, dw = nwaves * COST_DL;
    const int nr = 64 + dw - 1, nl = 64;
    const size_t need = (size_t)2 * (nr + nl) * es * 4 + (cost_tstore_shape(cn, nwaves) ? (size_t)2 * 64 * (nwaves + 1) * 16 : 0);
    return (cn == 3 && nwaves == 8 && need < CAMD_COST_LDS_FLOOR_RGB) ? (size_t)CAMD_COST_LDS_FLOOR_RGB : need;
}

typedef uint32_t u32x4_t __attribute__((ext_vector_type(4)));
#define KEEP_B128(q) asm volatile("" ::"v"(q))

constexpr int cost_min_waves(int K) { return K >= 11 ? 4 : (K >= 9 ? 5 : CAMD_COST_MIN_WAVES); }

template <int CN, int K, bool SAT>
__device__ __forceinline__ void cost_body(const uint8_t* __restrict__ left, const uint8_t* __restrict__ right,
                                          size_t pitch, size_t image_stride, uint16_t* __restrict__ Cout,
                                          const Geom& g, int rb, int nchunks, size_t vol_stride, const CostRanges& cr,
                                          uint32_t* __restrict__ ovf, int ovf_thresh, uint32_t* __restrict__ neg,
                                          const int bx, const int by, const int bz)
{
    constexpr int ES = CN == 1 ? 4 : 12;
    constexpr int EV = ES / 4;
    constexpr int DL = COST_DL;
    constexpr int NP = DL / 2;
    constexpr int SW2 = K / 2;
    constexpr int XS = 64 - (K - 1);
    constexpr bool NOCARRY = K * K * CN * (2 * CAMD_MAX_FTZERO + 63) + CAMD_MAX_P2 <= 65535;
    extern __shared__ uint4 cs_lds[];

    const int lane = threadIdx.x & 63, w = threadIdx.x >> 6, NW = blockDim.x >> 6, DW = NW * DL;
    const int tid = threadIdx.x;
    const int chunk = by % nchunks, dblk = by / nchunks;
    const int vpair = bz, pair = __builtin_amdgcn_readfirstlane(vpair / cr.n), ridx = __builtin_amdgcn_readfirstlane(vpair % cr.n);
    const int ybase = __builtin_amdgcn_readfirstlane(cr.start[ridx]), nrows = __builtin_amdgcn_readfirstlane(cr.rows[ridx]);
    if (chunk * rb >= nrows) return;
    if (SAT && ovf && !ovf[vpair]) return;
    uint32_t ovf_max = 0;
    uint32_t neg_min = SENT_PK;
    const int W1 = g.W1, H = g.H;
    const int xo0 = bx * XS, xs0 = xo0 - SW2;
    const int cmin = max(xs0, 0), cmax = min(xs0 + 63, W1 - 1);
    const int cx = min(max(xs0 + lane, 0), W1 - 1);
    const int db = dblk * DW;
    const int NL = cmax - cmin + 1, NR = NL + DW - 1;
    const int lcol0 = cmin + g.minX1;
    const int rcol0 = cmin + g.minX1 - g.minD - (db + DW - 1);
    const int NRmax = 64 + DW - 1, NLmax = 64;
    const int esz = (NRmax + NLmax) * EV;
    uint4* const Ebuf = cs_lds;

    const uint8_t* imgL = left + (size_t)pair * image_stride;
    const uint8_t* imgR = right + (size_t)pair * image_stride;
    const int ftz = g.ftzero;
    const uint32_t ftz2 = (uint32_t)ftz | ((uint32_t)ftz << 16);

    const int y0 = chunk * rb, y1 = min(y0 + rb, nrows);
    const int nsteps = (y1 - y0) + K - 1;
    auto row_of = [&](int r) { return min(max(ybase + y0 - SW2 + r, ybase), H - 1); };

    int st_k = 0, st_lo = 0, st_hi = 0, st_img = -1, st_total = 0;
    {
        int v = 0;
        for (int sg = 0; sg < 2; sg++) {
            const int n = sg ? NL : NR;
            for (int e = 0; e < n;) {
                int room = 64 - (v & 63);
                if (room < 5) { v += room; room = 64; }
                const int len = min(n - e, room - 4);
                if (tid >= v && tid < v + len + 4) { st_img = sg; st_k = e + (tid - v) - 2; st_lo = e; st_hi = e + len; }
                v += len + 4;
                e += len;
            }
        }
        st_total = v;
    }
    if (db + w * DL >= g.D && w * 64 >= st_total) return;
    const bool stager = st_img >= 0;
    const bool st_store = stager && st_k >= st_lo && st_k < st_hi;
    const int st_col = (st_img == 1 ? lcol0 : rcol0) + st_k;
    const bool st_inside = st_col > 0 && st_col < g.W - 1;
    const int st_ccol = min(max(st_col, 0), g.W - 1);
    const bool st_last = CN == 3 && st_ccol == g.W - 1;
    const uint32_t st_off = (uint32_t)(st_ccol * CN - (st_last ? 1 : 0));
    const uint32_t st_shift = st_last ? 8u : 0u;
    uint4* const st_dst = Ebuf + (st_img == 1 ? NRmax * EV : 0) + st_k * EV;

    uint32_t rowA = 0, rowB = 0, rowC = 0;
    auto fetch_rows = [&](int y) {
        if (stager) {
            const size_t om = (size_t)(y > 0 ? y - 1 : y) * pitch, o0 = (size_t)y * pitch, op = (size_t)(y < H - 1 ? y + 1 : y) * pitch;
            auto row_of_img = [&](const uint8_t* row) -> uint32_t {
                const __amdgpu_buffer_rsrc_t rs = __builtin_amdgcn_make_buffer_rsrc(const_cast<uint8_t*>(row), 0, 0x7fffffff, 0x00020000);
                if (CN == 1) return __builtin_amdgcn_raw_buffer_load_b8(rs, st_off, 0, 0);
                return __builtin_amdgcn_raw_buffer_load_b32(rs, st_off, 0, 0);
            };
            auto rows_of = [&](const uint8_t* img) {
                rowA = row_of_img(img + om);
                rowB = row_of_img(img + o0);
                rowC = row_of_img(img + op);
            };
            if (st_img == 1) {
                rows_of(imgL);
                asm volatile("; left image rows" ::: "memory");
            } else {
                rows_of(imgR);
                asm volatile("; right image rows" ::: "memory");
            }
        }
    };
    static_assert(2 * CAMD_MAX_FTZERO <= 255, "v_lerp_u8 halves 8-bit fields: a clipped gradient + ftzero must fit one");
    const uint32_t st_keep = st_inside ? 0xffffffffu : 0u, st_fill = st_inside ? 0u : ftz2;
    const uint32_t clip_lo = dup16(1024u - (uint32_t)ftz), clip_hi = dup16(1024u + (uint32_t)ftz);
    auto stage_entries = [&](int buf) {
        if (stager) {
            uint32_t u[CN], lo[CN], hi[CN];
            const uint32_t a = rowA >> st_shift, b = rowB >> st_shift, c = rowC >> st_shift;
            uint32_t vc[2];
#pragma unroll
            for (int eo = 0; eo < (CN == 1 ? 1 : 2); eo++) {
                const uint32_t M = CN == 1 ? 0xffu : 0x00ff00ffu;
                const uint32_t ea = (eo ? a >> 8 : a) & M, eb = (eo ? b >> 8 : b) & M, ec = (eo ? c >> 8 : c) & M;
                const uint32_t sv = ea + ec + eb + eb;
                uint32_t sl = dpp_perm<DPP_WAVE_SHR1>(sv);
                asm volatile("" : "+v"(sl));
                const uint32_t gq = dpp_perm<DPP_WAVE_SHL1>(sv) - sl + 0x04000400u;
                vc[eo] = pk_min_u16(pk_max_u16(gq, clip_lo), clip_hi) - clip_lo;
            }
#pragma unroll
            for (int ch = 0; ch < CN; ch++) {
                const uint32_t sel = ch == 0 ? 0x0c040100u : (ch == 1 ? 0x0c050100u : 0x0c060302u);
                u[ch] = (__builtin_amdgcn_perm(b, vc[ch & 1], sel) & st_keep) | st_fill;
            }
#pragma unroll
            for (int ch = 0; ch < CN; ch++) {
                const uint32_t l = dpp_perm<DPP_WAVE_SHR1>(u[ch]), r = dpp_perm<DPP_WAVE_SHL1>(u[ch]);
                lo[ch] = __builtin_amdgcn_lerp(u[ch], pk_min_u16(pk_min_u16(l, r), u[ch]), 0u);
                hi[ch] = __builtin_amdgcn_lerp(u[ch], pk_max_u16(pk_max_u16(l, r), u[ch]), 0u);
            }
            if (st_store) {
                u32x4_t* d4 = reinterpret_cast<u32x4_t*>(st_dst + buf * esz);
                if (CN == 1) {
                    d4[0] = u32x4_t{u[0], lo[0], hi[0], 0u};
                } else {
                    d4[0] = u32x4_t{u[0], lo[0], hi[0], u[1 % CN]};
                    d4[1] = u32x4_t{lo[1 % CN], hi[1 % CN], u[2 % CN], lo[2 % CN]};
                    d4[2] = u32x4_t{hi[2 % CN], 0u, 0u, 0u};
                }
            }
        }
    };

    fetch_rows(row_of(0));
    stage_entries(0);
    fetch_rows(row_of(1));
    __syncthreads();

    const int d0 = db + w * DL;
    const int d0u = db + __builtin_amdgcn_readfirstlane(w) * DL;
    uint32_t keep[NP];
#pragma unroll
    for (int k = 0; k < NP; k++)
        keep[k] = (d0u + 2 * k < g.D ? 0xffffu : 0u) | (d0u + 2 * k + 1 < g.D ? 0xffff0000u : 0u);
    const uint32_t rawmask = 0xfffcffffu;
    int eoff_l = NRmax * EV + (cx - cmin) * EV;
    int eoff_r = ((cx - cmin) + DW - 1 - w * DL - (DL - 1)) * EV;
    asm volatile("" : "+v"(eoff_l), "+v"(eoff_r));
    const int xo = xo0 + lane - (K - 1);
    const bool writer = lane >= K - 1 && xo < W1 && d0 < g.Dp;
    const bool first_col = xo == 0;
    uint16_t* const vol = Cout + (size_t)vpair * vol_stride;
    const uint32_t out_off = (uint32_t)((writer ? xo : 0) * g.Dp + d0);

    const uint32_t p2 = dup16((uint32_t)g.P2);
    const bool tstore = cost_tstore(CN) && 64 % NW == 0 && db + DW <= g.D;
    const int TP = NW + 1;
    uint4* const Tbuf = Ebuf + 2 * esz;
    const int tpx = w * (64 / NW) + lane / NW, tpc = lane % NW;
    const int txo = xo0 + tpx - (K - 1);
    const bool twriter = tpx >= K - 1 && txo < W1 && db + tpc * DL < g.Dp;
    const uint32_t tout_off = (uint32_t)((twriter ? txo : 0) * g.Dp + db + tpc * DL);
    auto store_c = [&](uint16_t* row, uint32_t off, u32x4_t v) {
        const __amdgpu_buffer_rsrc_t rs = __builtin_amdgcn_make_buffer_rsrc(row, 0, 0x7fffffff, 0x00020000);
        __builtin_amdgcn_raw_buffer_store_b128(v, rs, off * 2u, 0, 0);
    };
    auto flush_row = [&](int r) {
        if (twriter) {
            const uint4 v = Tbuf[((r & 1) * 64 + tpx) * TP + tpc];
            store_c(vol + (size_t)(y0 + r - (K - 1)) * W1 * g.Dp, tout_off, u32x4_t{v.x, v.y, v.z, v.w});
        }
    };
    uint32_t acc[NP], ring[K][NP];
#pragma unroll
    for (int k = 0; k < NP; k++) acc[k] = p2;
#pragma unroll
    for (int u = 0; u < K; u++)
#pragma unroll
        for (int k = 0; k < NP; k++) ring[u][k] = 0;

    for (int r0 = 0; r0 < nsteps; r0 += K) {
#pragma unroll
        for (int u = 0; u < K; u++) {
            const int r = r0 + u;
            if (r < nsteps) {
                if (tstore && r >= K) flush_row(r - 1);
                const uint4* E4 = Ebuf + (r & 1) * esz;
                uint32_t U[CN], U0[CN], U1[CN];
                {
                    const u32x4_t* q = reinterpret_cast<const u32x4_t*>(E4 + eoff_l);
                    if (CN == 1) {
                        const u32x4_t a = q[0];
                        U[0] = a.x; U0[0] = a.y; U1[0] = a.z;
                    } else {
                        const u32x4_t a = q[0], b = q[1], c = q[2];
                        KEEP_B128(c);
                        U[0] = a.x; U0[0] = a.y; U1[0] = a.z;
                        U[1 % CN] = a.w; U0[1 % CN] = b.x; U1[1 % CN] = b.y;
                        U[2 % CN] = b.z; U0[2 % CN] = b.w; U1[2 % CN] = c.x;
                    }
                }
                uint32_t cost[DL];
#pragma unroll
                for (int j = 0; j < DL; j++) {
                    const u32x4_t* q = reinterpret_cast<const u32x4_t*>(E4 + eoff_r + (DL - 1 - j) * EV);
                    uint32_t V[CN], V0[CN], V1[CN];
                    if (CN == 1) {
                        const u32x4_t a = q[0];
                        V[0] = a.x; V0[0] = a.y; V1[0] = a.z;
                    } else {
                        const u32x4_t a = q[0], b = q[1], c = q[2];
                        KEEP_B128(c);
                        V[0] = a.x; V0[0] = a.y; V1[0] = a.z;
                        V[1 % CN] = a.w; V0[1 % CN] = b.x; V1[1 % CN] = b.y;
                        V[2 % CN] = b.z; V0[2 % CN] = b.w; V1[2 % CN] = c.x;
                    }
                    uint32_t a32 = 0;
#pragma unroll
                    for (int c = 0; c < CN; c++) {
                        const uint32_t a = (pk_subsat_u16(U[c], V1[c]) | pk_subsat_u16(V0[c], U[c])) & rawmask;
                        const uint32_t b = (pk_subsat_u16(V[c], U1[c]) | pk_subsat_u16(U0[c], V[c])) & rawmask;
                        a32 += pk_min_u16(a, b);
                    }
                    cost[j] = a32;
                }
                uint32_t pp[NP];
#pragma unroll
                for (int k = 0; k < NP; k++) {
                    const uint32_t gq = __builtin_amdgcn_perm(cost[2 * k + 1], cost[2 * k], 0x05040100u);
                    const uint32_t rq = __builtin_amdgcn_perm(cost[2 * k + 1], cost[2 * k], 0x07060302u);
                    pp[k] = (gq + (rq >> 2)) & keep[k];
                }
#pragma unroll
                for (int k = 0; k < NP; k++) {
                    const uint32_t T = lane_window_sum<K>(pp[k]);
                    const uint32_t old = ring[u][k];
                    ring[u][k] = T;
                    if (SAT) {
                        const uint32_t a0 = pk_subsat_i16(pk_addsat_i16(acc[k], T), old);
                        const uint32_t a1 = pk_addsat_i16(pk_subsat_i16(acc[k], old), T);
                        acc[k] = (first_col && ybase + y0 + r - (K - 1) + SW2 < H) ? a0 : a1;
                    } else {
                        acc[k] = NOCARRY ? acc[k] + T - old : pk_sub_u16(pk_add_u16(acc[k], T), old);
                    }
                }
                if (tstore && r >= K - 1) Tbuf[((r & 1) * 64 + lane) * TP + w] = make_uint4(acc[0], acc[1], acc[2], acc[3]);
                if (r >= K - 1 && writer) {
                    const int y = y0 + r - (K - 1);
                    uint16_t* const orow = vol + (size_t)y * W1 * g.Dp;
#pragma unroll
                    for (int q = 0; q < NP / 4; q++) {
                        if (!tstore) store_c(orow, out_off + 8 * q, u32x4_t{acc[4 * q], acc[4 * q + 1], acc[4 * q + 2], acc[4 * q + 3]});
                        if (SAT) neg_min = pk_min_i16(pk_min_i16(neg_min, pk_min_i16(acc[4 * q], acc[4 * q + 1])),
                                                      pk_min_i16(acc[4 * q + 2], acc[4 * q + 3]));
                        if (!SAT && ovf_thresh >= 0)
                            ovf_max = pk_max_u16(pk_max_u16(ovf_max, pk_max_u16(acc[4 * q], acc[4 * q + 1])),
                                                 pk_max_u16(acc[4 * q + 2], acc[4 * q + 3]));
                    }
                }
#if defined(CAMD_COST_DBG_NOSTAGE) && !defined(CAMD_MEASUREMENT_BUILD)
#error "CAMD_COST_DBG_NOSTAGE produces wrong results: measurement builds only (define CAMD_MEASUREMENT_BUILD too)"
#endif
#ifndef CAMD_COST_DBG_NOSTAGE
                stage_entries((r + 1) & 1);
                fetch_rows(row_of(r + 2));
#endif
                __syncthreads();
            }
        }
    }
    if (tstore) flush_row(nsteps - 1);
    if (!SAT && ovf_thresh >= 0 && (int)max(ovf_max & 0xffffu, ovf_max >> 16) > ovf_thresh) atomicOr(ovf + vpair, 1u);
    if (SAT && neg && min((int)(int16_t)(neg_min & 0xffffu), (int)(int16_t)(neg_min >> 16)) < g.P2) atomicOr(neg + vpair, 1u);
}

template <int CN, int K, bool SAT>
__global__ __launch_bounds__(1024, cost_min_waves(K)) void k_cost(const uint8_t* __restrict__ left, const uint8_t* __restrict__ right,
                                               size_t pitch, size_t image_stride, uint16_t* __restrict__ Cout,
                                               Geom g, int rb, int nchunks, size_t vol_stride, CostRanges cr,
                                               uint32_t* __restrict__ ovf, int ovf_thresh, uint32_t* __restrict__ neg)
{
    cost_body<CN, K, SAT>(left, right, pitch, image_stride, Cout, g, rb, nchunks, vol_stride, cr, ovf, ovf_thresh, neg,
                          (int)blockIdx.x, (int)blockIdx.y, (int)blockIdx.z);
}

template <int CN, int K>
__global__ __launch_bounds__(1024, cost_min_waves(K)) void k_cost_persist(const uint8_t* __restrict__ left, const uint8_t* __restrict__ right,
                                               size_t pitch, size_t image_stride, uint16_t* __restrict__ Cout,
                                               Geom g, int rb, int nchunks, size_t vol_stride, CostRanges cr,
                                               uint32_t* __restrict__ ticket, int nx, int ny, int nitems)
{
    __shared__ int s_item;
    for (;;) {
        if (threadIdx.x == 0) s_item = (int)atomicAdd(ticket, 1u);
        __syncthreads();
        const int item = s_item;
        __syncthreads();
        if (item >= nitems) break;
        const int bx = item % nx, r = item / nx;
        cost_body<CN, K, false>(left, right, pitch, image_stride, Cout, g, rb, nchunks, vol_stride, cr, nullptr, -1, nullptr,
                                bx, r % ny, r / ny);
    }
}

}
```

### calibrating_amd/csrc/sgbm_exact.hpp

```cpp
#pragma once

namespace camd {

__global__ __launch_bounds__(256) void k_flag_below(const int16_t* __restrict__ C, Geom g, size_t vol_stride,
                                                    CostRanges cr, uint32_t* __restrict__ neg)
{
    const int vp = blockIdx.z, rows = cr.rows[vp % cr.n];
    const size_t n8 = (size_t)rows * g.W1 * (g.Dp / 8);
    const uint4* p = reinterpret_cast<const uint4*>(C + (size_t)vp * vol_stride);
    const uint32_t thr = dup16((uint32_t)g.P2);
    bool below = false;
    const int dq = g.Dp / 8;
    for (size_t i = (size_t)blockIdx.x * 256 + threadIdx.x; i < n8; i += (size_t)gridDim.x * 256) {
        uint4 q = p[i];
        const int d0 = (int)(i % (size_t)dq) * 8;
        if (d0 + 8 > g.D) {
            uint32_t* w = &q.x;
#pragma unroll
            for (int k = 0; k < 4; k++) {
                const int d = d0 + 2 * k;
                if (d >= g.D) w[k] = thr;
                else if (d + 1 >= g.D) w[k] = (w[k] & 0xffffu) | (thr & 0xffff0000u);
            }
        }
        const s16x2_t t = __builtin_bit_cast(s16x2_t, thr);
        const s16x2_t m = __builtin_elementwise_min(
            __builtin_elementwise_min(__builtin_bit_cast(s16x2_t, q.x), __builtin_bit_cast(s16x2_t, q.y)),
            __builtin_elementwise_min(__builtin_bit_cast(s16x2_t, q.z), __builtin_bit_cast(s16x2_t, q.w)));
        below |= m.x < t.x || m.y < t.y;
    }
    if (__any(below) && (threadIdx.x & 63) == 0) atomicOr(neg + vp, 1u);
}

template <int LANES>
__device__ __forceinline__ int group_min_i32(int v)
{
    if (LANES >= 2) v = min(v, (int)dpp_mov<DPP_QUAD_XOR1>((uint32_t)v, (uint32_t)v));
    if (LANES >= 4) v = min(v, (int)dpp_mov<DPP_QUAD_XOR2>((uint32_t)v, (uint32_t)v));
    if (LANES >= 8) v = min(v, (int)dpp_mov<DPP_ROW_HALF_MIRROR>((uint32_t)v, (uint32_t)v));
    if (LANES >= 16) v = min(v, (int)dpp_mov<DPP_ROW_MIRROR>((uint32_t)v, (uint32_t)v));
    return v;
}

__device__ __forceinline__ int sat16i(int v) { return v < -32768 ? -32768 : (v > 32767 ? 32767 : v); }

template <int LANES, int NR, bool STORE_SAT>
__device__ __forceinline__ void scan_exact_unit(const int16_t* __restrict__ Cv, int32_t* __restrict__ Lout, const Geom& g,
                                                const ScanDirs& sd, int dir, int unit, int min_as_int)
{
    constexpr int NE = 2 * NR;
    const int dx = sd.dx[dir], dy = sd.dy[dir], nlines = sd.nlines[dir];
    int32_t* __restrict__ Lv = Lout + (size_t)dir * sd.dir_stride;
    const int tid = unit * 256 + threadIdx.x;
    const int line = tid / LANES, li = tid % LANES;
    if (line >= nlines) return;
    const int W1 = g.W1, H = g.H;
    int x0, y0;
    if (dy == 0) {
        y0 = line;
        x0 = dx > 0 ? 0 : W1 - 1;
    } else {
        const int ys = dy > 0 ? 0 : H - 1;
        if (dx == 0 || line < W1) {
            x0 = line;
            y0 = ys;
        } else {
            x0 = dx > 0 ? 0 : W1 - 1;
            const int k = line - W1 + 1;
            y0 = dy > 0 ? k : H - 1 - k;
        }
    }
    const int lx = dx == 0 ? (1 << 30) : (dx > 0 ? W1 - x0 : x0 + 1);
    const int ly = dy == 0 ? (1 << 30) : (dy > 0 ? H - y0 : y0 + 1);
    const int len = min(lx, ly);
    const size_t off = ((size_t)y0 * W1 + x0) * g.Dp + (size_t)li * NE;
    const ptrdiff_t step = ((ptrdiff_t)dy * W1 + dx) * (ptrdiff_t)g.Dp;
    const int16_t* cp = Cv + off;
    int32_t* lp_out = Lv + off;
    const int dbase = li * NE;

    int Lp[NE];
#pragma unroll
    for (int j = 0; j < NE; j++) Lp[j] = 0;
    int minLp = 0;
    auto load8 = [&](const int16_t* p, int (&dst)[NE]) {
        uint32_t w[NR];
        ld_regs<NR>(reinterpret_cast<const uint16_t*>(p), w);
#pragma unroll
        for (int k = 0; k < NR; k++) {
            dst[2 * k] = (int)(int16_t)(w[k] & 0xffffu);
            dst[2 * k + 1] = (int)(int16_t)(w[k] >> 16);
        }
    };
    int c[NE], cn[NE];
    load8(cp, c);
    for (int i = 0; i < len; i++) {
        if (i + 1 < len) load8(cp + (ptrdiff_t)(i + 1) * step, cn);
        int left = (int)dpp_mov<DPP_ROW_SHR1>((uint32_t)MAX_COST, (uint32_t)Lp[NE - 1]);
        int right = (int)dpp_mov<DPP_ROW_SHL1>((uint32_t)MAX_COST, (uint32_t)Lp[0]);
        if (li == 0) left = MAX_COST;
        if (li == LANES - 1) right = MAX_COST;
        const int delta = minLp + g.P2;
        int L[NE], Lint[NE], mn = 0x7fffffff;
#pragma unroll
        for (int j = 0; j < NE; j++) {
            const int d = dbase + j;
            const int lm = d == 0 ? MAX_COST : (j == 0 ? left : Lp[j > 0 ? j - 1 : 0]);
            const int lq = d >= g.D - 1 ? MAX_COST : (j == NE - 1 ? right : Lp[j < NE - 1 ? j + 1 : j]);
            const int v = c[j] + min(min(lm + g.P1, lq + g.P1), min(Lp[j], delta)) - delta;
            const int st = STORE_SAT ? sat16i(v) : (int)(int16_t)v;
            L[j] = d < g.D ? st : 0;
            Lint[j] = d < g.D ? v : 0;
            if (d < g.D) mn = min(mn, STORE_SAT ? st : v);
        }
        mn = group_min_i32<LANES>(mn);
        minLp = (STORE_SAT || min_as_int) ? mn : (int)(int16_t)mn;
        int2* o = reinterpret_cast<int2*>(lp_out + (ptrdiff_t)i * step);
#pragma unroll
        for (int v = 0; v < NR; v++) o[v] = make_int2(Lint[2 * v], Lint[2 * v + 1]);
#pragma unroll
        for (int j = 0; j < NE; j++) { Lp[j] = L[j]; c[j] = cn[j]; }
    }
}

struct ExactArgs {
    const int16_t* C;
    int32_t* Lx;
    int16_t* dst;
    size_t vol_stride;
    size_t dst_stride_e;
    size_t dst_pitch_e;
    size_t dst_n;
    const uint32_t* neg;
    uint32_t* bar;
    uint32_t* err;
    int nvol, nd, tie_lanes, combine, min_as_int, invalid;
};
static constexpr uint32_t EXACT_SPIN_LIMIT = 1u << 23;

template <int LANES, int NR, bool STORE_SAT>
__global__ __launch_bounds__(256) void k_exact_all(ExactArgs a, Geom g, ScanDirs sd)
{
    uint32_t target = 0;
    bool dead = false;
    auto grid_sync = [&]() {
        __syncthreads();
        if (threadIdx.x == 0) {
            __threadfence();
            target += gridDim.x;
            atomicAdd(a.bar, 1u);
            uint32_t spins = 0;
            while (!dead && __hip_atomic_load(a.bar, __ATOMIC_RELAXED, __HIP_MEMORY_SCOPE_AGENT) < target) {
                __builtin_amdgcn_s_sleep(8);
                if (++spins > EXACT_SPIN_LIMIT) {
                    atomicOr(a.err, 4u);
                    dead = true;
                }
            }
            __threadfence();
        }
        __syncthreads();
    };
    int units[8], total = 0;
#pragma unroll
    for (int d = 0; d < 8; d++) {
        units[d] = d < a.nd ? (sd.nlines[d] * LANES + 255) / 256 : 0;
        total += units[d];
    }
    bool any = false;
    for (int vp = 0; vp < a.nvol; vp++) {
        if (!a.neg[vp]) continue;
        any = true;
        const int16_t* C = a.C + (size_t)vp * a.vol_stride;
        for (int u = blockIdx.x; u < total; u += gridDim.x) {
            int dir = 0, rest = u;
            while (rest >= units[dir]) rest -= units[dir++];
            scan_exact_unit<LANES, NR, STORE_SAT>(C, a.Lx, g, sd, dir, rest, a.min_as_int);
        }
        grid_sync();
        for (int y = blockIdx.x; y < g.H; y += gridDim.x) {
            wta_row<LANES, NR, true>(reinterpret_cast<const uint16_t*>(a.Lx), a.dst + (size_t)vp * a.dst_stride_e, a.dst_pitch_e,
                                     (size_t)0, g, (size_t)0, a.nd, sd.dir_stride, a.tie_lanes, a.combine, y, 0);
            __syncthreads();
        }
        grid_sync();
    }
    if (any && (__hip_atomic_load(a.err, __ATOMIC_RELAXED, __HIP_MEMORY_SCOPE_AGENT) & 4u)) {
        for (int vp = 0; vp < a.nvol; vp++) {
            if (!a.neg[vp]) continue;
            for (size_t i = (size_t)blockIdx.x * 256 + threadIdx.x; i < a.dst_n; i += (size_t)gridDim.x * 256)
                a.dst[(size_t)vp * a.dst_stride_e + i] = (int16_t)a.invalid;
        }
    }
}

}
```

Before: 1549 pairs/s.

## Store cost volume in interleaved disparity order for band SGM passes

Adds an interleaved disparity layout for the cost volume. Each 32-bit register pair now holds disparities d and d+NR rather than d and d+1, so the SGM step's neighbour (d±1) terms mostly come from adjacent registers and need no alignbit shifts. The cost kernel writes this order and the band, WTA, flag and exact kernels read it. A conversion kernel restores natural order for volume export. This adds index remapping and template instantiations, and rejects paths that cannot read the new layout.

Result: no change. 1555 pairs/s, median of 6 (+0.4%).

```diff
diff --git a/calibrating_amd/csrc/common.hpp b/calibrating_amd/csrc/common.hpp
--- a/calibrating_amd/csrc/common.hpp
+++ b/calibrating_amd/csrc/common.hpp
@@ -8,6 +8,7 @@
 
 #include "../../include/calibrating_amd.h"
 #include "../../include/calibrating_amd_experimental.h"
+#include "sgbm_layout.hpp"
 
 namespace camd {
 
diff --git a/calibrating_amd/csrc/sgbm.hip b/calibrating_amd/csrc/sgbm.hip
--- a/calibrating_amd/csrc/sgbm.hip
+++ b/calibrating_amd/csrc/sgbm.hip
@@ -67,6 +67,7 @@
     bool band_ok;
     int path;
     int keep_S;
+    bool vol_ilv;
     int cost_path;
     int saturate;
     int phases;
@@ -236,6 +237,8 @@
         }                                         \
     } while (0)
 
+static bool band_interleaved_shape(const Geom& g) { return g.lanes == 16 && 2 * g.nr == COST_DL; }
+
 static int invalid_disp(const Geom& g) { return (g.minD - 1) * 16; }
 
 static const int kDirs8[8][2] = {{1, 0}, {1, 1}, {0, 1}, {-1, 1}, {-1, 0}, {1, -1}, {0, -1}, {-1, -1}};
@@ -306,9 +309,19 @@
     CAMD_HIP(hipMemsetAsync(h->ticket, 0, 4, st));
     dim3 grid(full ? h->nbands * batch : div_up((long long)batch * g.H, BAND_THREADS / g.lanes)), block(BAND_BLOCK);
     const bool pad = g.Dp != g.D;
+    const bool ilv = h->vol_ilv;
+    if (ilv && (!band_interleaved_shape(g) || tie8 || mode == 1)) {
+        set_error("the volumes are in the interleaved order, which this band pass is not instantiated for");
+        return CAMD_ERR_UNSUPPORTED;
+    }
 #define CAMD_BAND(LN, NRR, FF, MM, DG)                                                                          \
     do {                                                                                                        \
-        if (pad || (NRR) % 4 != 0) hipLaunchKernelGGL((k_band<LN, NRR, FF, MM, true, DG>), grid, block, 0, st, a, g); \
+        constexpr bool IL = (LN) == 16 && (NRR) == 4;                                                           \
+        if (ilv && IL) {                                                                                        \
+            if (pad) hipLaunchKernelGGL((k_band<LN, NRR, FF, MM, true, DG, false, IL>), grid, block, 0, st, a, g);  \
+            else hipLaunchKernelGGL((k_band<LN, NRR, FF, MM, false, DG, false, IL>), grid, block, 0, st, a, g);     \
+        }                                                                                                       \
+        else if (pad || (NRR) % 4 != 0) hipLaunchKernelGGL((k_band<LN, NRR, FF, MM, true, DG>), grid, block, 0, st, a, g); \
         else hipLaunchKernelGGL((k_band<LN, ((NRR) % 4 ? 4 : (NRR)), FF, MM, false, DG>), grid, block, 0, st, a, g);   \
     } while (0)
 #define CAMD_BAND_F0T(LN, NRR) CAMD_BAND(LN, NRR, true, 0, true)
@@ -336,7 +349,11 @@
     }
     else if (!full && mode == 2 && h->persist_row > 0 && g.lanes == 16 && g.nr == 4) {
         const dim3 pgrid(h->persist_row * (h->num_cus > 0 ? h->num_cus : 256));
-        if (pad) hipLaunchKernelGGL((k_band_row_persist<16, 4, true>), pgrid, block, 0, st, a, g);
+        if (ilv) {
+            if (pad) hipLaunchKernelGGL((k_band_row_persist<16, 4, true, false, true>), pgrid, block, 0, st, a, g);
+            else hipLaunchKernelGGL((k_band_row_persist<16, 4, false, false, true>), pgrid, block, 0, st, a, g);
+        }
+        else if (pad) hipLaunchKernelGGL((k_band_row_persist<16, 4, true>), pgrid, block, 0, st, a, g);
         else hipLaunchKernelGGL((k_band_row_persist<16, 4, false>), pgrid, block, 0, st, a, g);
     }
     else if (!full && mode == 2) CAMD_FOR_BAND_SHAPE(g, CAMD_BAND_R2);
@@ -351,6 +368,13 @@
 #undef CAMD_BAND
     CAMD_LAUNCH_CHECK();
     return CAMD_OK;
+}
+
+__global__ __launch_bounds__(256) void k_vol_natural(const uint16_t* __restrict__ src, uint16_t* __restrict__ dst, size_t n,
+                                                     int Dp, int nr)
+{
+    const size_t i = (size_t)blockIdx.x * 256 + threadIdx.x;
+    if (i < n) dst[i] = src[vol_natural_src(i, Dp, nr)];
 }
 
 __global__ __launch_bounds__(256) void k_poison_flagged(int16_t* __restrict__ raw, size_t stride_e, size_t n,
@@ -391,6 +415,7 @@
     a.combine = g.mode == CAMD_MODE_HH4 ? 1 : (way3 ? 2 : 0);
     a.min_as_int = g.mode == CAMD_MODE_HH4 ? 1 : 0;
     a.invalid = invalid_disp(g);
+    a.ilv = h->vol_ilv ? 1 : 0;
     CAMD_HIP(hipMemsetAsync(h->xbar, 0, 4, st));
     const size_t lds = align_up((size_t)g.W * 6, 16);
     const dim3 grid(h->num_cus > 0 ? h->num_cus : 256);
@@ -526,6 +551,7 @@
 static int launch_cost(camd_sgbm* h, const uint8_t* left, const uint8_t* right, size_t pitch, size_t image_stride,
                        int vbatch, bool sat_kernel, uint32_t* ovf, int thresh, hipStream_t st)
 {
+    const bool ilv = h->vol_ilv;
     const Geom& g = h->g;
     const int K = 2 * g.SW2 + 1;
     CostShape s = cost_launch_shape(h, vbatch, sat_kernel ? COST_SATURATING : COST_CHUNKED);
@@ -537,17 +563,20 @@
         uint32_t* tk = h->ticket + 3;
         const int nx = s.nstrips, ny = s.nchunks * s.ndblk, nitems = nx * ny * vbatch;
         const dim3 pgrid(h->persist_cost * (h->num_cus > 0 ? h->num_cus : 256));
-#define CAMD_COSTP(CNN, KK) hipLaunchKernelGGL((k_cost_persist<CNN, KK>), pgrid, block, s.lds, st, left, right, pitch, image_stride, \
-                                               h->C, g, s.rows_per_chunk, s.nchunks, h->vol_elems, h->cr, tk, nx, ny, nitems)
+#define CAMD_COSTP_L(CNN, KK, IL) hipLaunchKernelGGL((k_cost_persist<CNN, KK, IL>), pgrid, block, s.lds, st, left, right, pitch, image_stride, \
+                                                     h->C, g, s.rows_per_chunk, s.nchunks, h->vol_elems, h->cr, tk, nx, ny, nitems)
+#define CAMD_COSTP(CNN, KK) do { if (ilv) CAMD_COSTP_L(CNN, KK, true); else CAMD_COSTP_L(CNN, KK, false); } while (0)
         if (g.cn == 1) { if (K == 5) CAMD_COSTP(1, 5); else CAMD_COSTP(1, 3); }
         else { if (K == 5) CAMD_COSTP(3, 5); else CAMD_COSTP(3, 3); }
 #undef CAMD_COSTP
+#undef CAMD_COSTP_L
         CAMD_LAUNCH_CHECK();
         return CAMD_OK;
     }
-#define CAMD_COST(CNN, KK, SS)                                                                                          \
-    hipLaunchKernelGGL((k_cost<CNN, KK, SS>), grid, block, s.lds, st, left, right, pitch, image_stride, h->C, g,        \
+#define CAMD_COST_L(CNN, KK, SS, IL)                                                                                    \
+    hipLaunchKernelGGL((k_cost<CNN, KK, SS, IL>), grid, block, s.lds, st, left, right, pitch, image_stride, h->C, g,    \
                        s.rows_per_chunk, s.nchunks, h->vol_elems, h->cr, ovf, thresh, h->cost_neg)
+#define CAMD_COST(CNN, KK, SS) do { if (ilv) CAMD_COST_L(CNN, KK, SS, true); else CAMD_COST_L(CNN, KK, SS, false); } while (0)
 #define CAMD_COST_K(CNN)                                                                         \
     switch (K) {                                                                                 \
         case 1: CAMD_COST(CNN, 1, false); break;                                                 \
@@ -560,6 +589,7 @@
     if (g.cn == 1) { CAMD_COST_K(1) } else { CAMD_COST_K(3) }
 #undef CAMD_COST_K
 #undef CAMD_COST
+#undef CAMD_COST_L
     CAMD_LAUNCH_CHECK();
     return CAMD_OK;
 }
@@ -617,6 +647,8 @@
     return CAMD_OK;
 }
 
+static bool want_interleaved(const camd_sgbm* h, int batch, bool fused_cost);
+
 static int run_cost(camd_sgbm* h, const uint8_t* left, const uint8_t* right, size_t pitch, size_t image_stride, int batch,
                     hipStream_t st)
 {
@@ -628,6 +660,7 @@
     const int vbatch = batch * h->cr.n;
     const bool fused = K <= 11 && (h->cost_path != CAMD_COST_SPLIT || way3);
     const bool do_cost = (h->phases & 1) != 0;
+    if (do_cost) h->vol_ilv = want_interleaved(h, batch, fused);
     if (fused && do_cost) {
         const int tbound = K * g.cn * (2 * g.ftzero + 63);
         const bool two_stage = sat && (long long)K * tbound + g.P2 <= 65535;
@@ -648,7 +681,7 @@
     if (do_cost && may_overflow && !(fused && sat)) {
         if (!fused) CAMD_HIP(hipMemsetAsync(h->cost_neg, 0, (size_t)vbatch * 4, st));
         hipLaunchKernelGGL(k_flag_below, dim3(512, 1, vbatch), dim3(256), 0, st, reinterpret_cast<const int16_t*>(h->C),
-                           h->ga, h->vol_elems, h->cr, h->cost_neg);
+                           h->ga, h->vol_elems, h->cr, h->cost_neg, h->vol_ilv ? 1 : 0);
         CAMD_LAUNCH_CHECK();
     }
     return CAMD_OK;
@@ -675,6 +708,12 @@
     return path;
 }
 
+static bool want_interleaved(const camd_sgbm* h, int batch, bool fused_cost)
+{
+    return fused_cost && h->g.mode != CAMD_MODE_SGBM_3WAY && band_interleaved_shape(h->g) &&
+           choose_path(h, batch) == CAMD_PATH_BAND;
+}
+
 static bool way3_inline(const camd_sgbm* h) { return h->way3_simd_lanes == 1 || h->g.D % 8 == 0; }
 static bool stops_before_last_pass(const camd_sgbm* h, int path)
 {
@@ -693,6 +732,10 @@
     const Geom& g = h->g;
     const bool way3 = g.mode == CAMD_MODE_SGBM_3WAY;
     const int vbatch = batch * h->cr.n;
+    if (h->vol_ilv && (path != CAMD_PATH_BAND || way3)) {
+        set_error("the cost volume was built in the interleaved order of the band passes; this call's path cannot read it");
+        return CAMD_ERR_UNSUPPORTED;
+    }
     if (path == CAMD_PATH_BAND && way3) {
         if (way3_inline(h)) CAMD_TRY(launch_wta_init(h, h->ga, vbatch, st));
         CAMD_TRY(launch_band(h, +1, +1, true, 0, vbatch, st, false));
@@ -1088,7 +1131,12 @@
         }
         if (g.W1 <= 0) return CAMD_OK;
         const uint16_t* src = (which == 0 ? h->C : h->S) + (size_t)index * h->vol_elems;
-        CAMD_HIP(hipMemcpyAsync(dst, src, (size_t)g.H * g.W1 * g.Dp * 2, hipMemcpyDeviceToDevice, st));
+        const size_t n = (size_t)g.H * g.W1 * g.Dp;
+        if (h->vol_ilv) {
+            hipLaunchKernelGGL(k_vol_natural, dim3(div_up((long long)n, 256)), dim3(256), 0, st, src, (uint16_t*)dst, n, g.Dp, g.nr);
+            CAMD_LAUNCH_CHECK();
+        }
+        else CAMD_HIP(hipMemcpyAsync(dst, src, n * 2, hipMemcpyDeviceToDevice, st));
     } else if (which == 2) {
         CAMD_HIP(hipMemcpyAsync(dst, h->raw + (size_t)index * h->raw_stride, (size_t)g.H * g.W * 2,
                                 hipMemcpyDeviceToDevice, st));
diff --git a/calibrating_amd/csrc/sgbm_band.hpp b/calibrating_amd/csrc/sgbm_band.hpp
--- a/calibrating_amd/csrc/sgbm_band.hpp
+++ b/calibrating_amd/csrc/sgbm_band.hpp
@@ -40,7 +40,7 @@
     int write_S;
 };
 
-template <int LANES, int NR, bool PAD>
+template <int LANES, int NR, bool PAD, bool ILV = false>
 __device__ __forceinline__ uint32_t sgm_step(const uint32_t (&Lp)[NR], uint32_t delta, const uint32_t (&c)[NR],
                                              uint32_t (&L)[NR], const uint32_t (&keep)[NR],
                                              const uint32_t (&sent)[NR], uint32_t P1pk, uint32_t P2pk, int li,
@@ -53,15 +53,20 @@
         if (li == 0) prev_last = SENT_PK;
         if (li == LANES - 1) next_first = SENT_PK;
     }
+    static_assert(!ILV || (LANES == 16 && NR >= 2), "the interleaved order is for whole 16-lane rows");
     uint32_t m[NR + 1];
-    m[0] = alignbit16(Lp[0], prev_last);
-#pragma unroll
-    for (int k = 1; k < NR; k++) m[k] = alignbit16(Lp[k], Lp[k - 1]);
-    m[NR] = alignbit16(next_first, Lp[NR - 1]);
+    m[0] = alignbit16(ILV ? Lp[NR - 1] : Lp[0], prev_last);
+    if (!ILV) {
+#pragma unroll
+        for (int k = 1; k < NR; k++) m[k] = alignbit16(Lp[k], Lp[k - 1]);
+    }
+    m[NR] = alignbit16(next_first, ILV ? Lp[0] : Lp[NR - 1]);
     uint32_t mn = SENT_PK;
 #pragma unroll
     for (int k = 0; k < NR; k++) {
-        uint32_t t = pk_min_u16(m[k], m[k + 1]) + P1pk;
+        const uint32_t down = ILV ? (k == 0 ? m[0] : Lp[k > 0 ? k - 1 : 0]) : m[k];
+        const uint32_t up = ILV ? (k == NR - 1 ? m[NR] : Lp[k < NR - 1 ? k + 1 : k]) : m[k + 1];
+        uint32_t t = pk_min_u16(down, up) + P1pk;
         uint32_t l = c[k] - pk_subsat_u16(delta, pk_min_u16(Lp[k], t));
         if (PAD) l = (l & keep[k]) | sent[k];
         L[k] = l;
@@ -79,13 +84,14 @@
 #endif
 template <int LANES> struct WtaPad { static constexpr int Q = (LANES * 16) % 128 == 0 ? CAMD_WTA_PADQ : 0; };
 
-template <int LANES, int NR, bool TIE8 = false, int NTH = BAND_THREADS>
+template <int LANES, int NR, bool TIE8 = false, int NTH = BAND_THREADS, bool ILV = false>
 __device__ __forceinline__ void band_wta_step(const uint32_t (&s)[NR], const uint32_t (&dpk)[NR], uint4* wS,
                                               const Geom& g, int ctid, int grp, int li, int t, bool act,
                                               uint32_t& cap_key, uint32_t& cap_nb)
 {
     constexpr int NQ = (NR + 3) / 4;
     static_assert(!TIE8 || NR % 4 == 0, "the 8-slot tie rule needs whole groups of 8 disparities per lane");
+    static_assert(!(TIE8 && ILV), "the 8-slot tie rule walks the registers in natural order");
     uint32_t key = 0xffffffffu;
 #pragma unroll
     for (int k = 0; k < NR; k++) {
@@ -136,8 +142,9 @@
     const bool ok = act && minS < MAX_COST && __umul24((uint32_t)minfar, uq) >= __umul24((uint32_t)minS, 100u);
     const uint16_t* gs = reinterpret_cast<const uint16_t*>(wS + grp * GST);
     auto slot_of = [](int d) {
-        if (NQ == 1 && NR == 4) return d;
-        const int ln = d / (2 * NR), w = d - ln * (2 * NR);
+        const int e = vol_slot(d, NR, ILV);
+        if (NQ == 1 && NR == 4) return e;
+        const int ln = e / (2 * NR), w = e - ln * (2 * NR);
         return (w >> 3) * (WS_PLANE * 8) + ln * 8 + (w & 7);
     };
     const uint32_t Sm = gs[slot_of(max(best - 1, 0))], Sp = gs[slot_of(min(best + 1, LANES * 2 * NR - 1))];
@@ -178,7 +185,7 @@
     cap_key = WTA_NONE;
 }
 
-template <int LANES, int NR, bool FULL, int MODE, bool PAD, bool DIAG, bool TIE8, bool ALLW>
+template <int LANES, int NR, bool FULL, int MODE, bool PAD, bool DIAG, bool TIE8, bool ALLW, bool ILV>
 __device__ __forceinline__ void band_body(const BandArgs& a, const Geom& g, const int ticket)
 {
     static_assert(!(FULL && ALLW), "the wavefront pass keeps its helper wave");
@@ -223,9 +230,9 @@
     uint32_t keep[NR], sent[NR], dpk[NR];
 #pragma unroll
     for (int k = 0; k < NR; k++) {
-        int d0 = li * 2 * NR + 2 * k;
-        dpk[k] = (uint32_t)d0 | ((uint32_t)(d0 + 1) << 16);
-        uint32_t kp = (d0 < g.D ? 0xffffu : 0u) | (d0 + 1 < g.D ? 0xffff0000u : 0u);
+        const int dlo = vol_disp(li * 2 * NR + 2 * k, NR, ILV), dhi = vol_disp(li * 2 * NR + 2 * k + 1, NR, ILV);
+        dpk[k] = (uint32_t)dlo | ((uint32_t)dhi << 16);
+        uint32_t kp = (dlo < g.D ? 0xffffu : 0u) | (dhi < g.D ? 0xffff0000u : 0u);
         keep[k] = kp;
         sent[k] = ~kp & SENT_PK;
     }
@@ -423,19 +430,19 @@
                 for (int k = 0; k < NR; k++) s[k] = MODE != 0 ? sr[u][k] : 0u;
                 {
                     uint32_t L[NR];
-                    dH = sgm_step<LANES, NR, PAD>(LH, dH, cc, L, keep, sent, P1pk, P2pk, li, edge_lo, edge_hi);
+                    dH = sgm_step<LANES, NR, PAD, ILV>(LH, dH, cc, L, keep, sent, P1pk, P2pk, li, edge_lo, edge_hi);
 #pragma unroll
                     for (int k = 0; k < NR; k++) { LH[k] = L[k]; s[k] = pk_addsat_i16(s[k], L[k]); }
                 }
                 if (FULL) {
-                    dVo = sgm_step<LANES, NR, PAD>(Vin, dV, cc, LVo, keep, sent, P1pk, P2pk, li, edge_lo, edge_hi);
+                    dVo = sgm_step<LANES, NR, PAD, ILV>(Vin, dV, cc, LVo, keep, sent, P1pk, P2pk, li, edge_lo, edge_hi);
 #pragma unroll
                     for (int k = 0; k < NR; k++) s[k] = pk_addsat_i16(s[k], LVo[k]);
                     if (DIAG) {
-                        dDo = sgm_step<LANES, NR, PAD>(Din, dD, cc, LDo, keep, sent, P1pk, P2pk, li, edge_lo, edge_hi);
+                        dDo = sgm_step<LANES, NR, PAD, ILV>(Din, dD, cc, LDo, keep, sent, P1pk, P2pk, li, edge_lo, edge_hi);
 #pragma unroll
                         for (int k = 0; k < NR; k++) s[k] = pk_addsat_i16(s[k], LDo[k]);
-                        dAo = sgm_step<LANES, NR, PAD>(An, dAn, cc, LAo, keep, sent, P1pk, P2pk, li, edge_lo, edge_hi);
+                        dAo = sgm_step<LANES, NR, PAD, ILV>(An, dAn, cc, LAo, keep, sent, P1pk, P2pk, li, edge_lo, edge_hi);
 #pragma unroll
                         for (int k = 0; k < NR; k++) s[k] = pk_addsat_i16(s[k], LAo[k]);
                     }
@@ -451,7 +458,7 @@
                     else st_regs<NR>(Srow + cell_off(xi), s);
                 }
 #endif
-                if (MODE == 2) band_wta_step<LANES, NR, TIE8, NTH>(s, dpk, wS, g, ctid, grp, li, t, true, cap_key, cap_nb);
+                if (MODE == 2) band_wta_step<LANES, NR, TIE8, NTH, ILV>(s, dpk, wS, g, ctid, grp, li, t, true, cap_key, cap_nb);
             }
             if (MODE == 2 && ((t & (LANES - 1)) == LANES - 1 || t == nsteps - 1)) {
                 const int xc = xi - ((t & (LANES - 1)) - li);
@@ -501,16 +508,16 @@
     }
 }
 
-template <int LANES, int NR, bool FULL, int MODE, bool PAD, bool DIAG = true, bool TIE8 = false>
+template <int LANES, int NR, bool FULL, int MODE, bool PAD, bool DIAG = true, bool TIE8 = false, bool ILV = false>
 __global__ __launch_bounds__(BAND_BLOCK, NR <= 4 ? (FULL ? CAMD_BAND_MIN_WAVES : CAMD_BAND_ROW_MIN_WAVES) : 2) void k_band(BandArgs a, Geom g)
 {
     __shared__ uint32_t s_ticket;
     if (threadIdx.x == 0) s_ticket = atomicAdd(a.ticket, 1u);
     __syncthreads();
-    band_body<LANES, NR, FULL, MODE, PAD, DIAG, TIE8, false>(a, g, (int)s_ticket);
-}
-
-template <int LANES, int NR, bool PAD, bool TIE8 = false>
+    band_body<LANES, NR, FULL, MODE, PAD, DIAG, TIE8, false, ILV>(a, g, (int)s_ticket);
+}
+
+template <int LANES, int NR, bool PAD, bool TIE8 = false, bool ILV = false>
 __global__ __launch_bounds__(BAND_BLOCK, NR <= 4 ? CAMD_BAND_ROW_MIN_WAVES : 2) void k_band_row_persist(BandArgs a, Geom g)
 {
     __shared__ uint32_t s_ticket;
@@ -524,7 +531,7 @@
         const int ticket = (int)s_ticket;
         __syncthreads();
         if ((long long)ticket * (BAND_BLOCK / LANES) >= rows) break;
-        band_body<LANES, NR, false, 2, PAD, true, TIE8, true>(a, g, ticket);
+        band_body<LANES, NR, false, 2, PAD, true, TIE8, true, ILV>(a, g, ticket);
     }
 }
 
diff --git a/calibrating_amd/csrc/sgbm_cost.hpp b/calibrating_amd/csrc/sgbm_cost.hpp
--- a/calibrating_amd/csrc/sgbm_cost.hpp
+++ b/calibrating_amd/csrc/sgbm_cost.hpp
@@ -74,7 +74,7 @@
 
 constexpr int cost_min_waves(int K) { return K >= 11 ? 4 : (K >= 9 ? 5 : CAMD_COST_MIN_WAVES); }
 
-template <int CN, int K, bool SAT>
+template <int CN, int K, bool SAT, bool ILV>
 __device__ __forceinline__ void cost_body(const uint8_t* __restrict__ left, const uint8_t* __restrict__ right,
                                           size_t pitch, size_t image_stride, uint16_t* __restrict__ Cout,
                                           const Geom& g, int rb, int nchunks, size_t vol_stride, const CostRanges& cr,
@@ -222,7 +222,7 @@
     uint32_t keep[NP];
 #pragma unroll
     for (int k = 0; k < NP; k++)
-        keep[k] = (d0u + 2 * k < g.D ? 0xffffu : 0u) | (d0u + 2 * k + 1 < g.D ? 0xffff0000u : 0u);
+        keep[k] = (d0u + vol_disp(2 * k, NP, ILV) < g.D ? 0xffffu : 0u) | (d0u + vol_disp(2 * k + 1, NP, ILV) < g.D ? 0xffff0000u : 0u);
     const uint32_t rawmask = 0xfffcffffu;
     int eoff_l = NRmax * EV + (cx - cmin) * EV;
     int eoff_r = ((cx - cmin) + DW - 1 - w * DL - (DL - 1)) * EV;
@@ -307,8 +307,9 @@
                 uint32_t pp[NP];
 #pragma unroll
                 for (int k = 0; k < NP; k++) {
-                    const uint32_t gq = __builtin_amdgcn_perm(cost[2 * k + 1], cost[2 * k], 0x05040100u);
-                    const uint32_t rq = __builtin_amdgcn_perm(cost[2 * k + 1], cost[2 * k], 0x07060302u);
+                    const int ja = vol_disp(2 * k, NP, ILV), jb = vol_disp(2 * k + 1, NP, ILV);
+                    const uint32_t gq = __builtin_amdgcn_perm(cost[jb], cost[ja], 0x05040100u);
+                    const uint32_t rq = __builtin_amdgcn_perm(cost[jb], cost[ja], 0x07060302u);
                     pp[k] = (gq + (rq >> 2)) & keep[k];
                 }
 #pragma unroll
@@ -354,17 +355,17 @@
     if (SAT && neg && min((int)(int16_t)(neg_min & 0xffffu), (int)(int16_t)(neg_min >> 16)) < g.P2) atomicOr(neg + vpair, 1u);
 }
 
-template <int CN, int K, bool SAT>
+template <int CN, int K, bool SAT, bool ILV = false>
 __global__ __launch_bounds__(1024, cost_min_waves(K)) void k_cost(const uint8_t* __restrict__ left, const uint8_t* __restrict__ right,
                                                size_t pitch, size_t image_stride, uint16_t* __restrict__ Cout,
                                                Geom g, int rb, int nchunks, size_t vol_stride, CostRanges cr,
                                                uint32_t* __restrict__ ovf, int ovf_thresh, uint32_t* __restrict__ neg)
 {
-    cost_body<CN, K, SAT>(left, right, pitch, image_stride, Cout, g, rb, nchunks, vol_stride, cr, ovf, ovf_thresh, neg,
+    cost_body<CN, K, SAT, ILV>(left, right, pitch, image_stride, Cout, g, rb, nchunks, vol_stride, cr, ovf, ovf_thresh, neg,
                           (int)blockIdx.x, (int)blockIdx.y, (int)blockIdx.z);
 }
 
-template <int CN, int K>
+template <int CN, int K, bool ILV = false>
 __global__ __launch_bounds__(1024, cost_min_waves(K)) void k_cost_persist(const uint8_t* __restrict__ left, const uint8_t* __restrict__ right,
                                                size_t pitch, size_t image_stride, uint16_t* __restrict__ Cout,
                                                Geom g, int rb, int nchunks, size_t vol_stride, CostRanges cr,
@@ -378,7 +379,7 @@
         __syncthreads();
         if (item >= nitems) break;
         const int bx = item % nx, r = item / nx;
-        cost_body<CN, K, false>(left, right, pitch, image_stride, Cout, g, rb, nchunks, vol_stride, cr, nullptr, -1, nullptr,
+        cost_body<CN, K, false, ILV>(left, right, pitch, image_stride, Cout, g, rb, nchunks, vol_stride, cr, nullptr, -1, nullptr,
                                 bx, r % ny, r / ny);
     }
 }
diff --git a/calibrating_amd/csrc/sgbm_exact.hpp b/calibrating_amd/csrc/sgbm_exact.hpp
--- a/calibrating_amd/csrc/sgbm_exact.hpp
+++ b/calibrating_amd/csrc/sgbm_exact.hpp
@@ -3,7 +3,7 @@
 namespace camd {
 
 __global__ __launch_bounds__(256) void k_flag_below(const int16_t* __restrict__ C, Geom g, size_t vol_stride,
-                                                    CostRanges cr, uint32_t* __restrict__ neg)
+                                                    CostRanges cr, uint32_t* __restrict__ neg, int ilv)
 {
     const int vp = blockIdx.z, rows = cr.rows[vp % cr.n];
     const size_t n8 = (size_t)rows * g.W1 * (g.Dp / 8);
@@ -14,13 +14,12 @@
     for (size_t i = (size_t)blockIdx.x * 256 + threadIdx.x; i < n8; i += (size_t)gridDim.x * 256) {
         uint4 q = p[i];
         const int d0 = (int)(i % (size_t)dq) * 8;
-        if (d0 + 8 > g.D) {
+        if ((ilv ? d0 - d0 % (2 * g.nr) + 2 * g.nr : d0 + 8) > g.D) {
             uint32_t* w = &q.x;
 #pragma unroll
             for (int k = 0; k < 4; k++) {
-                const int d = d0 + 2 * k;
-                if (d >= g.D) w[k] = thr;
-                else if (d + 1 >= g.D) w[k] = (w[k] & 0xffffu) | (thr & 0xffff0000u);
+                if (vol_disp(d0 + 2 * k, g.nr, ilv != 0) >= g.D) w[k] = (w[k] & 0xffff0000u) | (thr & 0xffffu);
+                if (vol_disp(d0 + 2 * k + 1, g.nr, ilv != 0) >= g.D) w[k] = (w[k] & 0xffffu) | (thr & 0xffff0000u);
             }
         }
         const s16x2_t t = __builtin_bit_cast(s16x2_t, thr);
@@ -46,7 +45,7 @@
 
 template <int LANES, int NR, bool STORE_SAT>
 __device__ __forceinline__ void scan_exact_unit(const int16_t* __restrict__ Cv, int32_t* __restrict__ Lout, const Geom& g,
-                                                const ScanDirs& sd, int dir, int unit, int min_as_int)
+                                                const ScanDirs& sd, int dir, int unit, int min_as_int, bool ilv)
 {
     constexpr int NE = 2 * NR;
     const int dx = sd.dx[dir], dy = sd.dy[dir], nlines = sd.nlines[dir];
@@ -87,9 +86,10 @@
         uint32_t w[NR];
         ld_regs<NR>(reinterpret_cast<const uint16_t*>(p), w);
 #pragma unroll
-        for (int k = 0; k < NR; k++) {
-            dst[2 * k] = (int)(int16_t)(w[k] & 0xffffu);
-            dst[2 * k + 1] = (int)(int16_t)(w[k] >> 16);
+        for (int j = 0; j < NE; j++) {
+            const int sn = vol_slot(j, NR, false), si = vol_slot(j, NR, true);
+            const uint32_t hn = (sn & 1) ? w[sn / 2] >> 16 : w[sn / 2] & 0xffffu, hi = (si & 1) ? w[si / 2] >> 16 : w[si / 2] & 0xffffu;
+            dst[j] = (int)(int16_t)(ilv ? hi : hn);
         }
     };
     int c[NE], cn[NE];
@@ -135,6 +135,7 @@
     uint32_t* bar;
     uint32_t* err;
     int nvol, nd, tie_lanes, combine, min_as_int, invalid;
+    int ilv;
 };
 static constexpr uint32_t EXACT_SPIN_LIMIT = 1u << 23;
 
@@ -175,7 +176,7 @@
         for (int u = blockIdx.x; u < total; u += gridDim.x) {
             int dir = 0, rest = u;
             while (rest >= units[dir]) rest -= units[dir++];
-            scan_exact_unit<LANES, NR, STORE_SAT>(C, a.Lx, g, sd, dir, rest, a.min_as_int);
+            scan_exact_unit<LANES, NR, STORE_SAT>(C, a.Lx, g, sd, dir, rest, a.min_as_int, a.ilv != 0);
         }
         grid_sync();
         for (int y = blockIdx.x; y < g.H; y += gridDim.x) {
diff --git a/calibrating_amd/csrc/sgbm_layout.hpp b/calibrating_amd/csrc/sgbm_layout.hpp
--- /dev/null
+++ b/calibrating_amd/csrc/sgbm_layout.hpp
@@ -0,0 +1,31 @@
+#pragma once
+
+#include <cstddef>
+
+#if defined(__HIPCC__)
+#define CAMD_HD __host__ __device__
+#else
+#define CAMD_HD
+#endif
+
+namespace camd {
+
+CAMD_HD constexpr int vol_slot(int d, int nr, bool interleaved)
+{
+    if (!interleaved) return d;
+    const unsigned u = (unsigned)d, n = (unsigned)nr, w = u % (2 * n);
+    return (int)(u - w + 2 * (w % n) + w / n);
+}
+CAMD_HD constexpr int vol_disp(int slot, int nr, bool interleaved)
+{
+    if (!interleaved) return slot;
+    const unsigned u = (unsigned)slot, n = (unsigned)nr, w = u % (2 * n);
+    return (int)(u - w + (w >> 1) + (w & 1) * n);
+}
+CAMD_HD constexpr size_t vol_natural_src(size_t i, int Dp, int nr)
+{
+    const int d = (int)(i % (size_t)Dp);
+    return i - (size_t)d + (size_t)vol_slot(d, nr, true);
+}
+
+}
```
